# elfi-dev/elfi

Measured on NVIDIA H100. Metric: accepted particles/sec, higher is better.
Workload: dtype f64

## Files before the change

### elfi_b200/csrc/distance.cu

```cuda
#include <cstdlib>

#include "rowstream.cuh"

extern "C" int elfi_b200_colmoments_f64(elfi_b200_ctx* ctx, const double* S, int64_t ldS, int64_t B,
                                        int64_t D, double* out, void* stream);

namespace elfi {

struct DistParams {
    const double* obs;
    const double* W;
    double* d_out;
    uint32_t* mask;
    int K;
    int has_thr;
    const double* shift_src;
    double* mom_partial;
    const double* thr_dev;
    double thr[ELFI_B200_MAX_NESTED];
    __device__ __forceinline__ double threshold(int k) const {
        return thr_dev ? __ldg(thr_dev + k) : thr[k];
    }
};

__device__ __forceinline__ void dist_setup_shared(uint8_t* aux, const DistParams& p, int D,
                                                  bool weighted) {
    const int Dp = ((D + RS_BOX_COLS - 1) / RS_BOX_COLS) * RS_BOX_COLS;
    double* obs_s = reinterpret_cast<double*>(aux);
    for (int j = threadIdx.x; j < Dp; j += blockDim.x) obs_s[j] = j < D ? p.obs[j] : 0.0;
    if (weighted) {
        double* w_s = obs_s + Dp;
        for (int k = 0; k < p.K; ++k)
            for (int j = threadIdx.x; j < Dp; j += blockDim.x)
                w_s[size_t(k) * Dp + j] = j < D ? p.W[size_t(k) * D + j] : 0.0;
    }
}

template <int KMAX>
__device__ __forceinline__ void dist_finish(const DistParams& p, const double (&acc)[KMAX], int K,
                                            int64_t row, int64_t B, int lane) {
    bool ok = row < B;
    if (ok) {
#pragma unroll
        for (int k = 0; k < KMAX; ++k) {
            if (k < K) {
                const double d = sqrt(acc[k]);
                p.d_out[row * K + k] = d;
                if (p.has_thr) ok = ok && (d <= p.threshold(k));
            }
        }
    }
    if (p.mask != nullptr) {
        const uint32_t bits = __ballot_sync(0xffffffffu, ok && p.has_thr);
        if (lane == 0) p.mask[row >> 5] = bits;
    }
}

struct EuclidConsumer {
    typedef DistParams Params;
    static constexpr int PASSES = 1;
    const Params& p;
    const double* obs_s;
    double acc;

    static __device__ void setup_shared(uint8_t* aux, const Params& p, int D) {
        dist_setup_shared(aux, p, D, false);
    }
    __device__ EuclidConsumer(const Params& p_, const uint8_t* aux, int, int)
        : p(p_), obs_s(reinterpret_cast<const double*>(aux)), acc(0.0) {}
    __device__ __forceinline__ void begin_row() { acc = 0.0; }
    __device__ __forceinline__ void consume(int, int cg, const uint8_t* box_row, int sw) {
        const double2* o = reinterpret_cast<const double2*>(obs_s + cg * RS_BOX_COLS);
#pragma unroll
        for (int c = 0; c < 8; ++c) {
            const double2 v = *reinterpret_cast<const double2*>(box_row + ((c ^ sw) << 4));
            const double2 ob = o[c];
            const double d0 = __dsub_rn(v.x, ob.x);
            const double d1 = __dsub_rn(v.y, ob.y);
            acc = __dadd_rn(acc, __dmul_rn(d0, d0));
            acc = __dadd_rn(acc, __dmul_rn(d1, d1));
        }
    }
    __device__ __forceinline__ void end_row(int64_t row, int64_t B, int lane) {
        const double a1[1] = {acc};
        dist_finish<1>(p, a1, 1, row, B, lane);
    }
};

struct WeightedConsumer {
    typedef DistParams Params;
    static constexpr int PASSES = 1;
    const Params& p;
    const double* obs_s;
    const double* w_s;
    double acc;

    static __device__ void setup_shared(uint8_t* aux, const Params& p, int D) {
        dist_setup_shared(aux, p, D, true);
    }
    __device__ WeightedConsumer(const Params& p_, const uint8_t* aux, int D, int)
        : p(p_), obs_s(reinterpret_cast<const double*>(aux)), acc(0.0) {
        w_s = obs_s + ((D + RS_BOX_COLS - 1) / RS_BOX_COLS) * RS_BOX_COLS;
    }
    __device__ __forceinline__ void begin_row() { acc = 0.0; }
    __device__ __forceinline__ void consume(int, int cg, const uint8_t* box_row, int sw) {
        const double2* o = reinterpret_cast<const double2*>(obs_s + cg * RS_BOX_COLS);
        const double2* wv = reinterpret_cast<const double2*>(w_s + cg * RS_BOX_COLS);
#pragma unroll
        for (int c = 0; c < 8; ++c) {
            const double2 v = *reinterpret_cast<const double2*>(box_row + ((c ^ sw) << 4));
            const double2 ob = o[c];
            const double2 w = wv[c];
            const double d0 = __dsub_rn(v.x, ob.x);
            const double d1 = __dsub_rn(v.y, ob.y);
            acc = __dadd_rn(acc, __dmul_rn(w.x, __dmul_rn(d0, d0)));
            acc = __dadd_rn(acc, __dmul_rn(w.y, __dmul_rn(d1, d1)));
        }
    }
    __device__ __forceinline__ void end_row(int64_t row, int64_t B, int lane) {
        const double a1[1] = {acc};
        dist_finish<1>(p, a1, 1, row, B, lane);
    }
};

template <int KMAX>
struct NestedConsumer {
    typedef DistParams Params;
    static constexpr int PASSES = 1;
    const Params& p;
    const double* obs_s;
    const double* w_s;
    int Dp;
    double acc[KMAX];

    static __device__ void setup_shared(uint8_t* aux, const Params& p, int D) {
        dist_setup_shared(aux, p, D, true);
    }
    __device__ NestedConsumer(const Params& p_, const uint8_t* aux, int D, int)
        : p(p_), obs_s(reinterpret_cast<const double*>(aux)) {
        Dp = ((D + RS_BOX_COLS - 1) / RS_BOX_COLS) * RS_BOX_COLS;
        w_s = obs_s + Dp;
#pragma unroll
        for (int k = 0; k < KMAX; ++k) acc[k] = 0.0;
    }
    __device__ __forceinline__ void begin_row() {
#pragma unroll
        for (int k = 0; k < KMAX; ++k) acc[k] = 0.0;
    }
    __device__ __forceinline__ void consume(int, int cg, const uint8_t* box_row, int sw) {
        const double2* o = reinterpret_cast<const double2*>(obs_s + cg * RS_BOX_COLS);
        const int K = p.K;
#pragma unroll
        for (int c = 0; c < 8; ++c) {
            const double2 v = *reinterpret_cast<const double2*>(box_row + ((c ^ sw) << 4));
            const double2 ob = o[c];
            const double d0 = __dsub_rn(v.x, ob.x);
            const double d1 = __dsub_rn(v.y, ob.y);
            const double s0 = __dmul_rn(d0, d0);
            const double s1 = __dmul_rn(d1, d1);
#pragma unroll
            for (int k = 0; k < KMAX; ++k) {
                if (k < K) {
                    const double2 w = *reinterpret_cast<const double2*>(
                        w_s + size_t(k) * Dp + cg * RS_BOX_COLS + 2 * c);
                    acc[k] = __dadd_rn(acc[k], __dmul_rn(w.x, s0));
                    acc[k] = __dadd_rn(acc[k], __dmul_rn(w.y, s1));
                }
            }
        }
    }
    __device__ __forceinline__ void end_row(int64_t row, int64_t B, int lane) {
        dist_finish<KMAX>(p, acc, p.K, row, B, lane);
    }
};

template <int KMAX>
struct NestedMomentsConsumer : NestedConsumer<KMAX> {
    typedef NestedConsumer<KMAX> Base;
    typedef DistParams Params;
    static constexpr bool RS_TILE_INFO = true;
    static constexpr bool RS_FINISH = true;
    const double* shift_s;
    double* acc_s;
    int64_t row0, nrows;
    int D;

    static __host__ __device__ size_t aux_bytes(int64_t Dp, int64_t K, int warps = RS_WARPS) {
        return size_t(Dp) * 8 * (1 + K + 1 + 2 * warps);
    }
    static __device__ void setup_shared(uint8_t* aux, const Params& p, int D) {
        dist_setup_shared(aux, p, D, true);
        const int Dp = ((D + RS_BOX_COLS - 1) / RS_BOX_COLS) * RS_BOX_COLS;
        double* shift = reinterpret_cast<double*>(aux) + size_t(1 + p.K) * Dp;
        for (int j = threadIdx.x; j < Dp; j += blockDim.x) shift[j] = j < D ? p.shift_src[j] : 0.0;
        double* acc = shift + Dp;
        const int warps = blockDim.x >> 5;
        for (int j = threadIdx.x; j < 2 * warps * Dp; j += blockDim.x) acc[j] = 0.0;
    }
    __device__ NestedMomentsConsumer(const Params& p_, const uint8_t* aux, int D_, int lane)
        : Base(p_, aux, D_, lane), row0(0), nrows(0), D(D_) {
        shift_s = this->obs_s + size_t(1 + p_.K) * this->Dp;
        acc_s = const_cast<double*>(shift_s) + this->Dp + size_t(threadIdx.x >> 5) * 2 * this->Dp;
    }
    __device__ __forceinline__ void set_tile(int64_t r0, int64_t B) { row0 = r0; nrows = B; }
    __device__ __forceinline__ void consume(int pass, int cg, const uint8_t* box_row, int sw) {
        Base::consume(pass, cg, box_row, sw);
        const int lane = threadIdx.x & 31;
        const int c2 = lane & 7, h = lane >> 3;
        const uint8_t* box = box_row - lane * 128;
        const double2 sh = *reinterpret_cast<const double2*>(shift_s + cg * RS_BOX_COLS + 2 * c2);
        double s1x = 0.0, s1y = 0.0, s2x = 0.0, s2y = 0.0;
#pragma unroll
        for (int i = 0; i < 8; ++i) {
            const int r = h * 8 + i;
            const double2 v = *reinterpret_cast<const double2*>(box + r * 128 + ((c2 ^ i) << 4));
            if (row0 + r < nrows) {
                const double dx = v.x - sh.x, dy = v.y - sh.y;
                s1x += dx;
                s1y += dy;
                s2x = fma(dx, dx, s2x);
                s2y = fma(dy, dy, s2y);
            }
        }
#pragma unroll
        for (int o = 8; o <= 16; o <<= 1) {
            s1x += __shfl_xor_sync(0xffffffffu, s1x, o);
            s1y += __shfl_xor_sync(0xffffffffu, s1y, o);
            s2x += __shfl_xor_sync(0xffffffffu, s2x, o);
            s2y += __shfl_xor_sync(0xffffffffu, s2y, o);
        }
        if (lane < 8) {
            double2* a1 = reinterpret_cast<double2*>(acc_s + cg * RS_BOX_COLS + 2 * c2);
            double2* a2 = reinterpret_cast<double2*>(acc_s + this->Dp + cg * RS_BOX_COLS + 2 * c2);
            double2 t1 = *a1, t2 = *a2;
            t1.x += s1x; t1.y += s1y; t2.x += s2x; t2.y += s2y;
            *a1 = t1;
            *a2 = t2;
        }
    }
    __device__ __forceinline__ void finish(int64_t gw, int lane) {
        double* out = this->p.mom_partial + gw * 2 * int64_t(D);
        for (int j = lane; j < D; j += 32) {
            out[j] = acc_s[j];
            out[D + j] = acc_s[this->Dp + j];
        }
    }
};

__global__ void __launch_bounds__(1024)
colmoments_flush_kernel(const double* __restrict__ S, const double* __restrict__ partial,
                        int64_t nwarps, int64_t B, int64_t D, double* __restrict__ out) {
    __shared__ double r1[32][33], r2[32][33];
    const int tx = threadIdx.x, ty = threadIdx.y;
    const int64_t c = int64_t(blockIdx.x) * 32 + tx;
    double s1 = 0.0, s2 = 0.0;
    if (c < D)
        for (int64_t b = ty; b < nwarps; b += 32) {
            s1 += partial[(b * 2 + 0) * D + c];
            s2 += partial[(b * 2 + 1) * D + c];
        }
    r1[ty][tx] = s1;
    r2[ty][tx] = s2;
    __syncthreads();
    if (ty == 0 && c < D) {
        for (int k = 1; k < 32; ++k) { s1 += r1[k][tx]; s2 += r2[k][tx]; }
        const double n = double(B);
        out[c] = S[c] + s1 / n;
        out[D + c] = s2 - s1 * s1 / n;
    }
}

template <int KMAX>
static int fused_moments_warps(elfi_b200_ctx* ctx, int64_t Dp, int64_t K) {
    int warps = 12;
    if (const char* e = getenv("ELFI_B200_FUSED_WARPS")) warps = atoi(e);
    if (KMAX > 8 || warps != 12) return RS_WARPS;
    const size_t aux = NestedMomentsConsumer<KMAX>::aux_bytes(Dp, K, warps);
    return rs_pick_stages(ctx->smem_optin, aux, warps) >= 3 ? warps : RS_WARPS;
}

template <int KMAX>
static int launch_nested_moments(elfi_b200_ctx* ctx, const double* S, int64_t ldS, int64_t B,
                                 int64_t D, DistParams p, double* moments, cudaStream_t stream) {
    const int64_t Dp = ((D + RS_BOX_COLS - 1) / RS_BOX_COLS) * RS_BOX_COLS;
    const int warps = fused_moments_warps<KMAX>(ctx, Dp, p.K);
    const size_t aux = NestedMomentsConsumer<KMAX>::aux_bytes(Dp, p.K, warps);
    const int64_t ntiles = (B + RS_BOX_ROWS - 1) / RS_BOX_ROWS;
    int64_t ctas = (ntiles + warps - 1) / warps;
    if (ctas > ctx->sm_count) ctas = ctx->sm_count;
    const int64_t nwarps = ctas * warps;
    int rc;
    if constexpr (KMAX <= 8) {
        if (warps == 12)
            rc = rowstream_launch<NestedMomentsConsumer<KMAX>, 12>(ctx, S, ldS, B, D, aux, p, stream);
        else
            rc = rowstream_launch<NestedMomentsConsumer<KMAX>>(ctx, S, ldS, B, D, aux, p, stream);
    } else {
        rc = rowstream_launch<NestedMomentsConsumer<KMAX>>(ctx, S, ldS, B, D, aux, p, stream);
    }
    if (rc) return rc;
    colmoments_flush_kernel<<<unsigned((D + 31) / 32), dim3(32, 32), 0, stream>>>(
        S, p.mom_partial, nwarps, B, D, moments);
    ELFI_CUDA_OK(cudaGetLastError());
    return ELFI_B200_OK;
}

__global__ void __launch_bounds__(256)
dist_direct_kernel(const double* __restrict__ S, int64_t ld, int64_t B, int D, DistParams p) {
    const int64_t row = int64_t(blockIdx.x) * blockDim.x + threadIdx.x;
    const int lane = threadIdx.x & 31;
    const int K = p.K;
    bool ok = row < B;
    if (ok) {
        const double* r = S + row * ld;
        for (int k = 0; k < K; ++k) {
            double acc = 0.0;
            if (p.W != nullptr) {
                const double* w = p.W + size_t(k) * D;
                for (int j = 0; j < D; ++j) {
                    const double d = __dsub_rn(__ldg(r + j), __ldg(p.obs + j));
                    acc = __dadd_rn(acc, __dmul_rn(__ldg(w + j), __dmul_rn(d, d)));
                }
            } else {
                for (int j = 0; j < D; ++j) {
                    const double d = __dsub_rn(__ldg(r + j), __ldg(p.obs + j));
                    acc = __dadd_rn(acc, __dmul_rn(d, d));
                }
            }
            const double dist = sqrt(acc);
            p.d_out[row * K + k] = dist;
            if (p.has_thr) ok = ok && (dist <= p.threshold(k));
        }
    }
    if (p.mask != nullptr) {
        const uint32_t bits = __ballot_sync(0xffffffffu, ok && p.has_thr);
        if (lane == 0 && (row - lane) < B) p.mask[row >> 5] = bits;
    }
}

__global__ void __launch_bounds__(1024)
compact_mask_kernel(const uint32_t* __restrict__ mask, int64_t nwords, int64_t B,
                    int32_t* __restrict__ idx, int64_t* __restrict__ n_out) {
    __shared__ int64_t warp_sums[32];
    __shared__ int64_t base_s;
    const int tid = threadIdx.x;
    const int lane = tid & 31;
    const int wid = tid >> 5;
    const int64_t first = int64_t(blockIdx.x) * 1024;

    int64_t before = 0;
    for (int64_t w = tid; w < first; w += 1024) before += __popc(mask[w]);
    for (int o = 16; o > 0; o >>= 1) before += __shfl_xor_sync(0xffffffffu, before, o);
    if (lane == 0) warp_sums[wid] = before;
    __syncthreads();
    if (tid == 0) {
        int64_t t = 0;
        for (int i = 0; i < 32; ++i) t += warp_sums[i];
        base_s = t;
    }
    __syncthreads();
    const int64_t base = base_s;
    __syncthreads();

    const int64_t w = first + tid;
    const uint32_t bits = w < nwords ? mask[w] : 0u;
    const int cnt = __popc(bits);
    int incl = cnt;
    for (int o = 1; o < 32; o <<= 1) {
        const int t = __shfl_up_sync(0xffffffffu, incl, o);
        if (lane >= o) incl += t;
    }
    if (lane == 31) warp_sums[wid] = incl;
    __syncthreads();
    if (wid == 0) {
        int64_t v = warp_sums[lane];
        int64_t inc2 = v;
        for (int o = 1; o < 32; o <<= 1) {
            const int64_t t = __shfl_up_sync(0xffffffffu, inc2, o);
            if (lane >= o) inc2 += t;
        }
        warp_sums[lane] = inc2 - v;
        if (lane == 31 && blockIdx.x == gridDim.x - 1 && n_out != nullptr) *n_out = base + inc2;
    }
    __syncthreads();
    int64_t pos = base + warp_sums[wid] + (incl - cnt);
    if (idx != nullptr) {
        uint32_t b = bits;
        while (b) {
            const int bit = __ffs(b) - 1;
            b &= b - 1;
            idx[pos++] = int32_t(w * 32 + bit);
        }
    }
}

int launch_compact_mask(const uint32_t* mask, int64_t B, int32_t* idx, int64_t* n_out,
                        cudaStream_t stream) {
    const int64_t nwords = (B + 31) / 32;
    if (nwords == 0) {
        if (n_out) ELFI_CUDA_OK(cudaMemsetAsync(n_out, 0, sizeof(int64_t), stream));
        return ELFI_B200_OK;
    }
    const unsigned blocks = unsigned((nwords + 1023) / 1024);
    compact_mask_kernel<<<blocks, 1024, 0, stream>>>(mask, nwords, B, idx, n_out);
    ELFI_CUDA_OK(cudaGetLastError());
    return ELFI_B200_OK;
}

int launch_dist(elfi_b200_ctx* ctx, const double* S, int64_t ldS, int64_t B, int64_t D,
                const double* obs, const double* W, int64_t K, const double* thr_host,
                double* d_out, uint32_t* mask, cudaStream_t stream,
                const double* thr_dev = nullptr) {
    DistParams p;
    memset(&p, 0, sizeof(p));
    p.obs = obs;
    p.W = W;
    p.d_out = d_out;
    p.mask = mask;
    p.K = int(K);
    p.has_thr = thr_host != nullptr || thr_dev != nullptr;
    p.thr_dev = thr_dev;
    if (thr_host)
        for (int k = 0; k < K; ++k) p.thr[k] = thr_host[k];
    if (B == 0) return ELFI_B200_OK;

    const int64_t Dp = ((D + RS_BOX_COLS - 1) / RS_BOX_COLS) * RS_BOX_COLS;
    const bool use_tma = D >= RS_BOX_COLS && tma_compatible(S, ldS);
    if (use_tma) {
        const size_t aux = size_t(Dp) * 8 * (W ? (1 + K) : 1);
        if (rs_pick_stages(ctx->smem_optin, aux) >= 2) {
            if (W == nullptr) return rowstream_launch<EuclidConsumer>(ctx, S, ldS, B, D, aux, p, stream);
            if (K == 1) return rowstream_launch<WeightedConsumer>(ctx, S, ldS, B, D, aux, p, stream);
            if (K <= 2) return rowstream_launch<NestedConsumer<2>>(ctx, S, ldS, B, D, aux, p, stream);
            if (K <= 3) return rowstream_launch<NestedConsumer<3>>(ctx, S, ldS, B, D, aux, p, stream);
            if (K <= 4) return rowstream_launch<NestedConsumer<4>>(ctx, S, ldS, B, D, aux, p, stream);
            if (K <= 5) return rowstream_launch<NestedConsumer<5>>(ctx, S, ldS, B, D, aux, p, stream);
            if (K <= 6) return rowstream_launch<NestedConsumer<6>>(ctx, S, ldS, B, D, aux, p, stream);
            if (K <= 8) return rowstream_launch<NestedConsumer<8>>(ctx, S, ldS, B, D, aux, p, stream);
            if (K <= 16) return rowstream_launch<NestedConsumer<16>>(ctx, S, ldS, B, D, aux, p, stream);
            return rowstream_launch<NestedConsumer<32>>(ctx, S, ldS, B, D, aux, p, stream);
        }
    }
    const unsigned blocks = unsigned((B + 255) / 256);
    dist_direct_kernel<<<blocks, 256, 0, stream>>>(S, ldS, B, int(D), p);
    ELFI_CUDA_OK(cudaGetLastError());
    return ELFI_B200_OK;
}

struct MetricParams : DistParams {
    double pexp;
    const double* V;
};

template <int METRIC>
__device__ __forceinline__ double metric_term(double acc, double d, double pexp) {
    if (METRIC == ELFI_B200_METRIC_SQEUCLIDEAN) return __dadd_rn(acc, __dmul_rn(d, d));
    if (METRIC == ELFI_B200_METRIC_CITYBLOCK) return __dadd_rn(acc, fabs(d));
    if (METRIC == ELFI_B200_METRIC_CHEBYSHEV) return fabs(d) > acc ? fabs(d) : acc;
    return __dadd_rn(acc, pow(fabs(d), pexp));
}

template <int METRIC>
__device__ __forceinline__ double metric_value(double acc, double pexp) {
    return METRIC == ELFI_B200_METRIC_MINKOWSKI ? pow(acc, 1.0 / pexp) : acc;
}

template <int METRIC>
__device__ __forceinline__ void metric_finish(const MetricParams& p, double acc, int64_t row,
                                              int64_t B, int lane, bool whole_warp) {
    bool ok = row < B;
    if (ok) {
        const double d = metric_value<METRIC>(acc, p.pexp);
        p.d_out[row] = d;
        if (p.has_thr) ok = d <= p.threshold(0);
    }
    if (p.mask != nullptr) {
        const uint32_t bits = __ballot_sync(0xffffffffu, ok && p.has_thr);
        if (lane == 0 && (whole_warp || (row - lane) < B)) p.mask[row >> 5] = bits;
    }
}

template <int METRIC>
struct MetricConsumer {
    typedef MetricParams Params;
    static constexpr int PASSES = 1;
    const Params& p;
    const double* obs_s;
    double acc;

    static __device__ void setup_shared(uint8_t* aux, const Params& p, int D) {
        dist_setup_shared(aux, p, D, false);
    }
    __device__ MetricConsumer(const Params& p_, const uint8_t* aux, int, int)
        : p(p_), obs_s(reinterpret_cast<const double*>(aux)), acc(0.0) {}
    __device__ __forceinline__ void begin_row() { acc = 0.0; }
    __device__ __forceinline__ void consume(int, int cg, const uint8_t* box_row, int sw) {
        const double2* o = reinterpret_cast<const double2*>(obs_s + cg * RS_BOX_COLS);
#pragma unroll
        for (int c = 0; c < 8; ++c) {
            const double2 v = *reinterpret_cast<const double2*>(box_row + ((c ^ sw) << 4));
            const double2 ob = o[c];
            acc = metric_term<METRIC>(acc, __dsub_rn(v.x, ob.x), p.pexp);
            acc = metric_term<METRIC>(acc, __dsub_rn(v.y, ob.y), p.pexp);
        }
    }
    __device__ __forceinline__ void end_row(int64_t row, int64_t B, int lane) {
        metric_finish<METRIC>(p, acc, row, B, lane, true);
    }
};

template <int METRIC>
__global__ void __launch_bounds__(256)
metric_direct_kernel(const double* __restrict__ S, int64_t ld, int64_t B, int D, MetricParams p) {
    const int64_t row = int64_t(blockIdx.x) * blockDim.x + threadIdx.x;
    double acc = 0.0;
    if (row < B) {
        const double* r = S + row * ld;
        for (int j = 0; j < D; ++j)
            acc = metric_term<METRIC>(acc, __dsub_rn(__ldg(r + j), __ldg(p.obs + j)), p.pexp);
    }
    metric_finish<METRIC>(p, acc, row, B, threadIdx.x & 31, false);
}

template <int METRIC>
static int launch_metric_t(elfi_b200_ctx* ctx, const double* S, int64_t ldS, int64_t B, int64_t D,
                           const MetricParams& p, cudaStream_t stream) {
    const int64_t Dp = ((D + RS_BOX_COLS - 1) / RS_BOX_COLS) * RS_BOX_COLS;
    const size_t aux = size_t(Dp) * 8;
    if (D >= RS_BOX_COLS && tma_compatible(S, ldS) && rs_pick_stages(ctx->smem_optin, aux) >= 2)
        return rowstream_launch<MetricConsumer<METRIC>>(ctx, S, ldS, B, D, aux, p, stream);
    metric_direct_kernel<METRIC><<<unsigned((B + 255) / 256), 256, 0, stream>>>(S, ldS, B, int(D), p);
    ELFI_CUDA_OK(cudaGetLastError());
    return ELFI_B200_OK;
}

static int launch_metric(elfi_b200_ctx* ctx, int metric, double pexp, const double* S, int64_t ldS,
                         int64_t B, int64_t D, const double* obs, const double* thr_host,
                         double* d_out, uint32_t* mask, cudaStream_t stream) {
    MetricParams p;
    memset(&p, 0, sizeof(p));
    p.obs = obs;
    p.d_out = d_out;
    p.mask = mask;
    p.K = 1;
    p.has_thr = thr_host != nullptr;
    if (thr_host) p.thr[0] = thr_host[0];
    p.pexp = pexp;
    if (B == 0) return ELFI_B200_OK;
    switch (metric) {
        case ELFI_B200_METRIC_SQEUCLIDEAN:
            return launch_metric_t<ELFI_B200_METRIC_SQEUCLIDEAN>(ctx, S, ldS, B, D, p, stream);
        case ELFI_B200_METRIC_CITYBLOCK:
            return launch_metric_t<ELFI_B200_METRIC_CITYBLOCK>(ctx, S, ldS, B, D, p, stream);
        case ELFI_B200_METRIC_CHEBYSHEV:
            return launch_metric_t<ELFI_B200_METRIC_CHEBYSHEV>(ctx, S, ldS, B, D, p, stream);
        default:
            return launch_metric_t<ELFI_B200_METRIC_MINKOWSKI>(ctx, S, ldS, B, D, p, stream);
    }
}

struct SeuclidTerm {
    double even, odd, last;
    int j_last;
    __device__ __forceinline__ void begin(int D) {
        even = 0.0;
        odd = 0.0;
        last = 0.0;
        j_last = (D & 1) ? D - 1 : -1;
    }
    __device__ __forceinline__ void pair(int j0, double t0, double t1) {
        if (j0 == j_last) {
            last = t0;
        } else {
            even = __dadd_rn(even, t0);
            odd = __dadd_rn(odd, t1);
        }
    }
    __device__ __forceinline__ double value() const {
        const double s = __dadd_rn(even, odd);
        return sqrt(j_last >= 0 ? __dadd_rn(s, last) : s);
    }
};

__device__ __forceinline__ double seuclid_term(double x, double o, double v) {
    const double d = __dsub_rn(x, o);
    return __ddiv_rn(__dmul_rn(d, d), v);
}

__device__ __forceinline__ void seuclid_finish(const MetricParams& p, double dist, int64_t row,
                                               int64_t B, int lane, bool whole_warp) {
    bool ok = row < B;
    if (ok) {
        p.d_out[row] = dist;
        if (p.has_thr) ok = dist <= p.threshold(0);
    }
    if (p.mask != nullptr) {
        const uint32_t bits = __ballot_sync(0xffffffffu, ok && p.has_thr);
        if (lane == 0 && (whole_warp || (row - lane) < B)) p.mask[row >> 5] = bits;
    }
}

struct SeuclidConsumer {
    typedef MetricParams Params;
    static constexpr int PASSES = 1;
    const Params& p;
    const double* obs_s;
    const double* v_s;
    int D;
    SeuclidTerm acc;

    static __device__ void setup_shared(uint8_t* aux, const Params& p, int D) {
        const int Dp = ((D + RS_BOX_COLS - 1) / RS_BOX_COLS) * RS_BOX_COLS;
        double* obs_s = reinterpret_cast<double*>(aux);
        for (int j = threadIdx.x; j < Dp; j += blockDim.x) {
            obs_s[j] = j < D ? p.obs[j] : 0.0;
            obs_s[Dp + j] = j < D ? p.V[j] : 1.0;
        }
    }
    __device__ SeuclidConsumer(const Params& p_, const uint8_t* aux, int D_, int)
        : p(p_), obs_s(reinterpret_cast<const double*>(aux)), D(D_) {
        v_s = obs_s + ((D + RS_BOX_COLS - 1) / RS_BOX_COLS) * RS_BOX_COLS;
        acc.begin(D);
    }
    __device__ __forceinline__ void begin_row() { acc.begin(D); }
    __device__ __forceinline__ void consume(int, int cg, const uint8_t* box_row, int sw) {
        const double2* o = reinterpret_cast<const double2*>(obs_s + cg * RS_BOX_COLS);
        const double2* vv = reinterpret_cast<const double2*>(v_s + cg * RS_BOX_COLS);
#pragma unroll
        for (int c = 0; c < 8; ++c) {
            const double2 x = *reinterpret_cast<const double2*>(box_row + ((c ^ sw) << 4));
            const double2 ob = o[c];
            const double2 v = vv[c];
            acc.pair(cg * RS_BOX_COLS + 2 * c, seuclid_term(x.x, ob.x, v.x),
                     seuclid_term(x.y, ob.y, v.y));
        }
    }
    __device__ __forceinline__ void end_row(int64_t row, int64_t B, int lane) {
        seuclid_finish(p, acc.value(), row, B, lane, true);
    }
};

__global__ void __launch_bounds__(256)
seuclid_direct_kernel(const double* __restrict__ S, int64_t ld, int64_t B, int D, MetricParams p) {
    const int64_t row = int64_t(blockIdx.x) * blockDim.x + threadIdx.x;
    SeuclidTerm acc;
    acc.begin(D);
    if (row < B) {
        const double* r = S + row * ld;
        for (int j = 0; j < D; j += 2) {
            const double t0 = seuclid_term(__ldg(r + j), __ldg(p.obs + j), __ldg(p.V + j));
            const double t1 = j + 1 < D
                ? seuclid_term(__ldg(r + j + 1), __ldg(p.obs + j + 1), __ldg(p.V + j + 1)) : 0.0;
            acc.pair(j, t0, t1);
        }
    }
    seuclid_finish(p, acc.value(), row, B, threadIdx.x & 31, false);
}

static int launch_seuclid(elfi_b200_ctx* ctx, const double* S, int64_t ldS, int64_t B, int64_t D,
                          const double* obs, const double* V, const double* thr_host,
                          double* d_out, uint32_t* mask, cudaStream_t stream) {
    MetricParams p;
    memset(&p, 0, sizeof(p));
    p.obs = obs;
    p.V = V;
    p.d_out = d_out;
    p.mask = mask;
    p.K = 1;
    p.has_thr = thr_host != nullptr;
    if (thr_host) p.thr[0] = thr_host[0];
    if (B == 0) return ELFI_B200_OK;
    const int64_t Dp = ((D + RS_BOX_COLS - 1) / RS_BOX_COLS) * RS_BOX_COLS;
    const size_t aux = size_t(Dp) * 8 * 2;
    if (D >= RS_BOX_COLS && tma_compatible(S, ldS) && rs_pick_stages(ctx->smem_optin, aux) >= 2)
        return rowstream_launch<SeuclidConsumer>(ctx, S, ldS, B, D, aux, p, stream);
    seuclid_direct_kernel<<<unsigned((B + 255) / 256), 256, 0, stream>>>(S, ldS, B, int(D), p);
    ELFI_CUDA_OK(cudaGetLastError());
    return ELFI_B200_OK;
}

static int check_dist_args(const void* S, int64_t ldS, int64_t B, int64_t D, const void* obs,
                           const void* W, int64_t K, const void* thr, const void* acc_idx) {
    ELFI_REQUIRE(B >= 0 && D >= 1, "dist: bad shape B=%lld D=%lld", (long long)B, (long long)D);
    ELFI_REQUIRE(B == 0 || S != nullptr, "dist: S is NULL");
    ELFI_REQUIRE(obs != nullptr, "dist: obs is NULL");
    ELFI_REQUIRE(ldS >= D, "dist: ldS (%lld) < D (%lld)", (long long)ldS, (long long)D);
    ELFI_REQUIRE(K >= 1 && K <= ELFI_B200_MAX_NESTED, "dist: K=%lld outside [1, %d]",
                 (long long)K, ELFI_B200_MAX_NESTED);
    ELFI_REQUIRE(W != nullptr || K == 1, "dist: K=%lld needs a weight matrix", (long long)K);
    ELFI_REQUIRE(acc_idx == nullptr || thr != nullptr, "dist: acc_idx requires thresholds");
    ELFI_REQUIRE(B < (int64_t(1) << 31), "dist: B must fit int32 row indices");
    return ELFI_B200_OK;
}

}

extern "C" {

int elfi_b200_dist_euclid_thr_f64(elfi_b200_ctx* ctx, const double* S, int64_t ldS, int64_t B,
                                  int64_t D, const double* obs, const double* W, int64_t K,
                                  const double* thr_host, double* d_out, int32_t* acc_idx,
                                  int64_t* n_acc, void* stream_) {
    using namespace elfi;
    ELFI_REQUIRE(ctx != nullptr, "dist: ctx is NULL");
    int rc = check_dist_args(S, ldS, B, D, obs, W, K, thr_host, acc_idx);
    if (rc) return rc;
    ELFI_REQUIRE(B == 0 || d_out != nullptr, "dist: d_out is NULL");
    cudaStream_t stream = static_cast<cudaStream_t>(stream_);
    ELFI_CUDA_OK(cudaSetDevice(ctx->device));
    uint32_t* mask = nullptr;
    if (thr_host != nullptr) {
        const size_t nwords = size_t((B + 31) / 32);
        mask = static_cast<uint32_t*>(ctx_scratch(ctx, nwords * 4 + 256));
        if (!mask) return ELFI_B200_ERR_NOMEM;
    }
    rc = launch_dist(ctx, S, ldS, B, D, obs, W, K, thr_host, d_out, mask, stream);
    if (rc) return rc;
    if (thr_host != nullptr && (acc_idx != nullptr || n_acc != nullptr))
        return launch_compact_mask(mask, B, acc_idx, n_acc, stream);
    return ELFI_B200_OK;
}

int elfi_b200_dist_euclid_thr_dev_f64(elfi_b200_ctx* ctx, const double* S, int64_t ldS, int64_t B,
                                      int64_t D, const double* obs, const double* W, int64_t K,
                                      const double* thr_dev, double* d_out, int32_t* acc_idx,
                                      int64_t* n_acc, void* stream_) {
    using namespace elfi;
    ELFI_REQUIRE(ctx != nullptr && thr_dev != nullptr, "dist: ctx or thr_dev is NULL");
    int rc = check_dist_args(S, ldS, B, D, obs, W, K, thr_dev, acc_idx);
    if (rc) return rc;
    ELFI_REQUIRE(B == 0 || d_out != nullptr, "dist: d_out is NULL");
    cudaStream_t stream = static_cast<cudaStream_t>(stream_);
    ELFI_CUDA_OK(cudaSetDevice(ctx->device));
    const size_t nwords = size_t((B + 31) / 32);
    uint32_t* mask = static_cast<uint32_t*>(ctx_scratch(ctx, nwords * 4 + 256));
    if (!mask) return ELFI_B200_ERR_NOMEM;
    rc = launch_dist(ctx, S, ldS, B, D, obs, W, K, nullptr, d_out, mask, stream, thr_dev);
    if (rc) return rc;
    if (acc_idx != nullptr || n_acc != nullptr)
        return launch_compact_mask(mask, B, acc_idx, n_acc, stream);
    return ELFI_B200_OK;
}

int elfi_b200_dist_euclid_mom_f64(elfi_b200_ctx* ctx, const double* S, int64_t ldS, int64_t B,
                                  int64_t D, const double* obs, const double* W, int64_t K,
                                  const double* thr_host, const double* thr_dev, double* d_out,
                                  int32_t* acc_idx, int64_t* n_acc, double* moments,
                                  void* stream_) {
    using namespace elfi;
    ELFI_REQUIRE(ctx != nullptr && moments != nullptr, "dist_mom: ctx or moments is NULL");
    ELFI_REQUIRE(!(thr_host && thr_dev), "dist_mom: give thresholds on the host OR on the device");
    const void* thr = thr_host ? static_cast<const void*>(thr_host) : thr_dev;
    int rc = check_dist_args(S, ldS, B, D, obs, W, K, thr, acc_idx);
    if (rc) return rc;
    ELFI_REQUIRE(B >= 1 && d_out != nullptr, "dist_mom: needs at least one row and d_out");
    cudaStream_t stream = static_cast<cudaStream_t>(stream_);
    ELFI_CUDA_OK(cudaSetDevice(ctx->device));
    const int64_t Dp = ((D + RS_BOX_COLS - 1) / RS_BOX_COLS) * RS_BOX_COLS;
    const size_t aux = NestedMomentsConsumer<2>::aux_bytes(Dp, K);
    const bool fused = W != nullptr && D >= RS_BOX_COLS && tma_compatible(S, ldS) &&
                       rs_pick_stages(ctx->smem_optin, aux) >= 2;
    const size_t mask_bytes = (size_t((B + 31) / 32) * 4 + 255) & ~size_t(255);
    const size_t part_bytes = fused ? size_t(ctx->sm_count) * 16 * 2 * D * 8 : 0;
    uint8_t* base = static_cast<uint8_t*>(ctx_scratch(ctx, mask_bytes + part_bytes + 256));
    if (!base) return ELFI_B200_ERR_NOMEM;
    uint32_t* mask = thr ? reinterpret_cast<uint32_t*>(base) : nullptr;
    if (!fused) {
        rc = launch_dist(ctx, S, ldS, B, D, obs, W, K, thr_host, d_out, mask, stream, thr_dev);
        if (rc) return rc;
        if (thr && (acc_idx != nullptr || n_acc != nullptr)) {
            rc = launch_compact_mask(mask, B, acc_idx, n_acc, stream);
            if (rc) return rc;
        }
        return elfi_b200_colmoments_f64(ctx, S, ldS, B, D, moments, stream_);
    }
    DistParams p;
    memset(&p, 0, sizeof(p));
    p.obs = obs;
    p.W = W;
    p.d_out = d_out;
    p.mask = mask;
    p.K = int(K);
    p.has_thr = thr != nullptr;
    p.thr_dev = thr_dev;
    if (thr_host)
        for (int k = 0; k < K; ++k) p.thr[k] = thr_host[k];
    p.shift_src = S;
    p.mom_partial = reinterpret_cast<double*>(base + mask_bytes);
    if (K <= 2) rc = launch_nested_moments<2>(ctx, S, ldS, B, D, p, moments, stream);
    else if (K <= 4) rc = launch_nested_moments<4>(ctx, S, ldS, B, D, p, moments, stream);
    else if (K <= 6) rc = launch_nested_moments<6>(ctx, S, ldS, B, D, p, moments, stream);
    else if (K <= 8) rc = launch_nested_moments<8>(ctx, S, ldS, B, D, p, moments, stream);
    else if (K <= 16) rc = launch_nested_moments<16>(ctx, S, ldS, B, D, p, moments, stream);
    else rc = launch_nested_moments<32>(ctx, S, ldS, B, D, p, moments, stream);
    if (rc) return rc;
    if (thr && (acc_idx != nullptr || n_acc != nullptr))
        return launch_compact_mask(mask, B, acc_idx, n_acc, stream);
    return ELFI_B200_OK;
}

int elfi_b200_dist_euclid_thr_f64_host(elfi_b200_ctx* ctx, const double* S_host, int64_t ldS,
                                       int64_t B, int64_t D, const double* obs_host,
                                       const double* W_host, int64_t K, const double* thr_host,
                                       double* d_out_host, int32_t* acc_idx_host,
                                       int64_t* n_acc_host) {
    using namespace elfi;
    ELFI_REQUIRE(ctx != nullptr, "dist_host: ctx is NULL");
    int rc = check_dist_args(S_host, ldS, B, D, obs_host, W_host, K, thr_host, acc_idx_host);
    if (rc) return rc;
    ELFI_CUDA_OK(cudaSetDevice(ctx->device));

    const int64_t row_bytes = D * 8;
    int64_t chunk_rows = (int64_t(32) << 20) / row_bytes;
    chunk_rows = (chunk_rows / 32) * 32;
    if (chunk_rows < 32) chunk_rows = 32;
    if (chunk_rows > B) chunk_rows = ((B + 31) / 32) * 32;
    const size_t chunk_bytes = size_t(chunk_rows) * row_bytes;
    const size_t nwords = size_t((B + 31) / 32);
    auto align = [](size_t v) { return (v + 255) & ~size_t(255); };
    const size_t off_chunk1 = align(chunk_bytes);
    const size_t off_obs = off_chunk1 + align(chunk_bytes);
    const size_t off_w = off_obs + align(size_t(D) * 8);
    const size_t off_d = off_w + align(size_t(K) * D * 8);
    const size_t off_mask = off_d + align(size_t(B) * K * 8);
    const size_t off_idx = off_mask + align(nwords * 4 + 4);
    const size_t off_n = off_idx + align(size_t(B) * 4 + 4);
    const size_t total = off_n + 256;
    if (total > ctx->dev_stage_bytes) {
        ELFI_CUDA_OK(cudaDeviceSynchronize());
        if (ctx->dev_stage) ELFI_CUDA_OK(cudaFree(ctx->dev_stage));
        ctx->dev_stage = nullptr;
        ctx->dev_stage_bytes = 0;
        ELFI_CUDA_OK(cudaMalloc(&ctx->dev_stage, total));
        ctx->dev_stage_bytes = total;
    }
    uint8_t* base = static_cast<uint8_t*>(ctx->dev_stage);
    double* chunk[2] = {reinterpret_cast<double*>(base), reinterpret_cast<double*>(base + off_chunk1)};
    double* obs_d = reinterpret_cast<double*>(base + off_obs);
    double* w_d = W_host ? reinterpret_cast<double*>(base + off_w) : nullptr;
    double* d_d = reinterpret_cast<double*>(base + off_d);
    uint32_t* mask_d = thr_host ? reinterpret_cast<uint32_t*>(base + off_mask) : nullptr;
    int32_t* idx_d = reinterpret_cast<int32_t*>(base + off_idx);
    int64_t* n_d = reinterpret_cast<int64_t*>(base + off_n);

    cudaStream_t s0 = ctx->copy_stream[0], s1 = ctx->copy_stream[1];
    ELFI_CUDA_OK(cudaMemcpyAsync(obs_d, obs_host, size_t(D) * 8, cudaMemcpyHostToDevice, s0));
    if (W_host)
        ELFI_CUDA_OK(cudaMemcpyAsync(w_d, W_host, size_t(K) * D * 8, cudaMemcpyHostToDevice, s0));
    ELFI_CUDA_OK(cudaEventRecord(ctx->copy_event[0], s0));
    ELFI_CUDA_OK(cudaStreamWaitEvent(s1, ctx->copy_event[0], 0));

    int which = 0;
    for (int64_t r0 = 0; r0 < B; r0 += chunk_rows, which ^= 1) {
        const int64_t rows = (B - r0) < chunk_rows ? (B - r0) : chunk_rows;
        cudaStream_t st = which ? s1 : s0;
        if (ldS == D) {
            ELFI_CUDA_OK(cudaMemcpyAsync(chunk[which], S_host + r0 * ldS, size_t(rows) * row_bytes,
                                         cudaMemcpyHostToDevice, st));
        } else {
            ELFI_CUDA_OK(cudaMemcpy2DAsync(chunk[which], size_t(row_bytes), S_host + r0 * ldS,
                                           size_t(ldS) * 8, size_t(row_bytes), size_t(rows),
                                           cudaMemcpyHostToDevice, st));
        }
        rc = launch_dist(ctx, chunk[which], D, rows, D, obs_d, w_d, K, thr_host, d_d + r0 * K,
                         mask_d ? mask_d + r0 / 32 : nullptr, st);
        if (rc) return rc;
    }
    ELFI_CUDA_OK(cudaEventRecord(ctx->copy_event[1], s1));
    ELFI_CUDA_OK(cudaStreamWaitEvent(s0, ctx->copy_event[1], 0));
    ELFI_CUDA_OK(cudaEventRecord(ctx->copy_event[2], s0));
    ELFI_CUDA_OK(cudaStreamWaitEvent(s1, ctx->copy_event[2], 0));
    if (d_out_host && B > 0)
        ELFI_CUDA_OK(cudaMemcpyAsync(d_out_host, d_d, size_t(B) * K * 8, cudaMemcpyDeviceToHost, s1));
    int64_t n_acc = 0;
    if (thr_host != nullptr) {
        rc = launch_compact_mask(mask_d, B, acc_idx_host ? idx_d : nullptr, n_d, s0);
        if (rc) return rc;
        ELFI_CUDA_OK(cudaMemcpyAsync(&n_acc, n_d, 8, cudaMemcpyDeviceToHost, s0));
        ELFI_CUDA_OK(cudaStreamSynchronize(s0));
        if (acc_idx_host && n_acc > 0)
            ELFI_CUDA_OK(cudaMemcpyAsync(acc_idx_host, idx_d, size_t(n_acc) * 4,
                                         cudaMemcpyDeviceToHost, s0));
        if (n_acc_host) *n_acc_host = n_acc;
    }
    ELFI_CUDA_OK(cudaStreamSynchronize(s0));
    ELFI_CUDA_OK(cudaStreamSynchronize(s1));
    return ELFI_B200_OK;
}

int elfi_b200_dist_metric_thr_f64(elfi_b200_ctx* ctx, int32_t metric, double pexp, const double* S,
                                  int64_t ldS, int64_t B, int64_t D, const double* obs,
                                  const double* thr_host, double* d_out, int32_t* acc_idx,
                                  int64_t* n_acc, void* stream_) {
    using namespace elfi;
    ELFI_REQUIRE(ctx != nullptr, "dist_metric: ctx is NULL");
    ELFI_REQUIRE(metric >= ELFI_B200_METRIC_SQEUCLIDEAN && metric <= ELFI_B200_METRIC_MINKOWSKI,
                 "dist_metric: unknown metric code %d", int(metric));
    ELFI_REQUIRE(metric != ELFI_B200_METRIC_MINKOWSKI || (pexp > 0.0 && pexp < 1e308),
                 "dist_metric: Minkowski exponent must be positive and finite");
    int rc = check_dist_args(S, ldS, B, D, obs, nullptr, 1, thr_host, acc_idx);
    if (rc) return rc;
    ELFI_REQUIRE(B == 0 || d_out != nullptr, "dist_metric: d_out is NULL");
    cudaStream_t stream = static_cast<cudaStream_t>(stream_);
    ELFI_CUDA_OK(cudaSetDevice(ctx->device));
    uint32_t* mask = nullptr;
    if (thr_host != nullptr) {
        mask = static_cast<uint32_t*>(ctx_scratch(ctx, size_t((B + 31) / 32) * 4 + 256));
        if (!mask) return ELFI_B200_ERR_NOMEM;
    }
    rc = launch_metric(ctx, int(metric), pexp, S, ldS, B, D, obs, thr_host, d_out, mask, stream);
    if (rc) return rc;
    if (thr_host != nullptr && (acc_idx != nullptr || n_acc != nullptr))
        return launch_compact_mask(mask, B, acc_idx, n_acc, stream);
    return ELFI_B200_OK;
}

int elfi_b200_dist_seuclidean_thr_f64(elfi_b200_ctx* ctx, const double* S, int64_t ldS, int64_t B,
                                      int64_t D, const double* obs, const double* V,
                                      const double* thr_host, double* d_out, int32_t* acc_idx,
                                      int64_t* n_acc, void* stream_) {
    using namespace elfi;
    ELFI_REQUIRE(ctx != nullptr, "dist_seuclidean: ctx is NULL");
    ELFI_REQUIRE(V != nullptr, "dist_seuclidean: V is NULL");
    int rc = check_dist_args(S, ldS, B, D, obs, nullptr, 1, thr_host, acc_idx);
    if (rc) return rc;
    ELFI_REQUIRE(B == 0 || d_out != nullptr, "dist_seuclidean: d_out is NULL");
    cudaStream_t stream = static_cast<cudaStream_t>(stream_);
    ELFI_CUDA_OK(cudaSetDevice(ctx->device));
    uint32_t* mask = nullptr;
    if (thr_host != nullptr) {
        mask = static_cast<uint32_t*>(ctx_scratch(ctx, size_t((B + 31) / 32) * 4 + 256));
        if (!mask) return ELFI_B200_ERR_NOMEM;
    }
    rc = launch_seuclid(ctx, S, ldS, B, D, obs, V, thr_host, d_out, mask, stream);
    if (rc) return rc;
    if (thr_host != nullptr && (acc_idx != nullptr || n_acc != nullptr))
        return launch_compact_mask(mask, B, acc_idx, n_acc, stream);
    return ELFI_B200_OK;
}

}
```

### elfi_b200/csrc/rowstream.cuh

```cuda
#pragma once

#include <type_traits>

#include "common.cuh"

namespace elfi {

template <class C, class = void> struct rs_has_tile_info : std::false_type {};
template <class C> struct rs_has_tile_info<C, std::void_t<decltype(C::RS_TILE_INFO)>> : std::true_type {};
template <class C, class = void> struct rs_has_finish : std::false_type {};
template <class C> struct rs_has_finish<C, std::void_t<decltype(C::RS_FINISH)>> : std::true_type {};

constexpr int RS_WARPS = 8;
constexpr int RS_BOX_ROWS = 32;
constexpr int RS_BOX_COLS = 16;
constexpr int RS_BOX_BYTES = RS_BOX_ROWS * RS_BOX_COLS * 8;
constexpr int RS_MAX_STAGES = 6;

__host__ __device__ inline size_t rs_box_bytes(int ns, int warps = RS_WARPS) {
    return size_t(warps) * ns * RS_BOX_BYTES;
}
__host__ __device__ inline size_t rs_bar_bytes(int ns, int warps = RS_WARPS) {
    return size_t(warps) * ns * 8;
}
__host__ __device__ inline size_t rs_aux_offset(int ns, int warps = RS_WARPS) {
    return (rs_box_bytes(ns, warps) + rs_bar_bytes(ns, warps) + 15) & ~size_t(15);
}

inline int rs_pick_stages(size_t smem_optin, size_t aux_bytes, int warps = RS_WARPS) {
    for (int ns = RS_MAX_STAGES; ns >= 2; --ns)
        if (rs_aux_offset(ns, warps) + aux_bytes + 1024 <= smem_optin) return ns;
    return 0;
}

template <class Consumer, int WARPS = RS_WARPS>
__global__ void __launch_bounds__(WARPS * 32, 1)
rowstream_kernel(const __grid_constant__ CUtensorMap map, int64_t B, int D, int ns,
                 typename Consumer::Params params) {
    extern __shared__ __align__(1024) uint8_t smem[];
    const int warp = threadIdx.x >> 5;
    const int lane = threadIdx.x & 31;
    uint8_t* aux = smem + rs_aux_offset(ns, WARPS);

    Consumer::setup_shared(aux, params, D);

    const uint32_t box0 = smem_u32(smem) + uint32_t(warp) * ns * RS_BOX_BYTES;
    const uint32_t bar0 = smem_u32(smem + rs_box_bytes(ns, WARPS)) + uint32_t(warp) * ns * 8;
    const uint8_t* box0_generic = smem + size_t(warp) * ns * RS_BOX_BYTES;

    if (lane == 0) {
        if (warp == 0) tma_prefetch_desc(&map);
        for (int s = 0; s < ns; ++s) mbar_init(bar0 + s * 8, 1);
        mbar_fence_init();
    }
    __syncthreads();

    const int Gc = (D + RS_BOX_COLS - 1) / RS_BOX_COLS;
    const int G = Gc * Consumer::PASSES;
    const int64_t ntiles = (B + RS_BOX_ROWS - 1) / RS_BOX_ROWS;
    const int64_t gw = int64_t(blockIdx.x) * WARPS + warp;
    const int64_t GW = int64_t(gridDim.x) * WARPS;
    const int64_t my_tiles = gw < ntiles ? (ntiles - gw + GW - 1) / GW : 0;
    const int64_t nbox = my_tiles * G;

    int64_t p_tile = gw;
    int p_cg = 0;
    int p_col = 0;
    int64_t p_q = 0;
    int p_s = 0;
    auto issue = [&]() {
        mbar_arrive_expect_tx(bar0 + p_s * 8, RS_BOX_BYTES);
        tma_load_2d(box0 + p_s * RS_BOX_BYTES, &map, p_col * RS_BOX_COLS,
                    int32_t(p_tile * RS_BOX_ROWS), bar0 + p_s * 8);
        ++p_q;
        if (++p_s == ns) p_s = 0;
        if (++p_col == Gc) p_col = 0;
        if (++p_cg == G) { p_cg = 0; p_tile += GW; }
    };
    if (lane == 0) {
        const int64_t pre = nbox < ns ? nbox : ns;
        for (int64_t i = 0; i < pre; ++i) issue();
    }

    Consumer c(params, aux, D, lane);
    const int sw = lane & 7;
    const uint32_t row_off = uint32_t(lane) * 128;

    int s = 0;
    uint32_t parity = 0;
    int cg = 0;
    int col = 0;
    int pass = 0;
    int64_t tile = gw;
    for (int64_t q = 0; q < nbox; ++q) {
        mbar_wait(bar0 + s * 8, parity);
        if (cg == 0) {
            c.begin_row();
            if constexpr (rs_has_tile_info<Consumer>::value) c.set_tile(tile * RS_BOX_ROWS, B);
        }
        c.consume(pass, col, box0_generic + size_t(s) * RS_BOX_BYTES + row_off, sw);
        __syncwarp();
        if (lane == 0 && p_q < nbox) issue();
        if (cg == G - 1) c.end_row(tile * RS_BOX_ROWS + lane, B, lane);
        if (++col == Gc) { col = 0; ++pass; }
        if (++cg == G) { cg = 0; pass = 0; tile += GW; }
        if (++s == ns) { s = 0; parity ^= 1; }
    }
    if constexpr (rs_has_finish<Consumer>::value) {
        __syncwarp();
        c.finish(gw, lane);
    }
}

template <class Consumer, int WARPS = RS_WARPS>
int rowstream_launch(elfi_b200_ctx* ctx, const double* M, int64_t ld, int64_t B, int64_t D,
                     size_t aux_bytes, const typename Consumer::Params& params,
                     cudaStream_t stream) {
    ELFI_REQUIRE(D <= (int64_t(1) << 30) && B < (int64_t(1) << 31),
                 "matrix too large for int32 TMA coordinates (B=%lld, D=%lld)", (long long)B,
                 (long long)D);
    if (B == 0) return ELFI_B200_OK;
    const int ns = rs_pick_stages(ctx->smem_optin, aux_bytes, WARPS);
    ELFI_REQUIRE(ns >= 2, "row too wide for the shared-memory pipeline (D=%lld)", (long long)D);
    CUtensorMap map;
    int rc = make_rowmajor_f64_map(ctx, M, B, D, ld, RS_BOX_ROWS, &map);
    if (rc) return rc;
    const size_t smem_bytes = rs_aux_offset(ns, WARPS) + aux_bytes;
    auto kern = rowstream_kernel<Consumer, WARPS>;
    ELFI_CUDA_OK(cudaFuncSetAttribute(kern, cudaFuncAttributeMaxDynamicSharedMemorySize,
                                      int(smem_bytes)));
    const int64_t ntiles = (B + RS_BOX_ROWS - 1) / RS_BOX_ROWS;
    int64_t ctas = (ntiles + WARPS - 1) / WARPS;
    if (ctas > ctx->sm_count) ctas = ctx->sm_count;
    kern<<<dim3(unsigned(ctas)), dim3(WARPS * 32), smem_bytes, stream>>>(map, B, int(D), ns, params);
    ELFI_CUDA_OK(cudaGetLastError());
    return ELFI_B200_OK;
}

}
```

### elfi_b200/csrc/select.cu

```cuda
#include <cstdlib>

#include "eqweight.h"
#include "pairwise.cuh"

namespace elfi {

constexpr int SORT_CHUNK = 1024;
constexpr int SORT_WARPS = 8;

__device__ __forceinline__ uint64_t key_to_u64(double d) {
    if (d != d) return ~uint64_t(0);
    uint64_t u = static_cast<uint64_t>(__double_as_longlong(d));
    return (u >> 63) ? ~u : (u | (uint64_t(1) << 63));
}
__device__ __forceinline__ double u64_to_key(uint64_t u) {
    if (u == ~uint64_t(0)) return __longlong_as_double(0x7ff8000000000000LL);
    u = (u >> 63) ? (u & ~(uint64_t(1) << 63)) : ~u;
    return __longlong_as_double(static_cast<long long>(u));
}

__global__ void __launch_bounds__(256)
sort_prepare_kernel(const double* __restrict__ keys, int64_t n, uint64_t* __restrict__ ukeys,
                    int32_t* __restrict__ vals, uint32_t* __restrict__ ghist) {
    __shared__ uint32_t h[8 * 256];
    for (int i = threadIdx.x; i < 8 * 256; i += blockDim.x) h[i] = 0;
    __syncthreads();
    const int64_t stride = int64_t(gridDim.x) * blockDim.x;
    for (int64_t i = int64_t(blockIdx.x) * blockDim.x + threadIdx.x; i < n; i += stride) {
        const uint64_t u = key_to_u64(keys[i]);
        ukeys[i] = u;
        vals[i] = int32_t(i);
#pragma unroll
        for (int p = 0; p < 8; ++p) atomicAdd(&h[p * 256 + ((u >> (8 * p)) & 255)], 1u);
    }
    __syncthreads();
    for (int i = threadIdx.x; i < 8 * 256; i += blockDim.x)
        if (h[i]) atomicAdd(&ghist[i], h[i]);
}

__device__ __forceinline__ bool pass_trivial(const uint32_t* ghist, int pass, int64_t n,
                                             uint64_t first_key) {
    return ghist[pass * 256 + ((first_key >> (8 * pass)) & 255)] == uint32_t(n);
}

__global__ void __launch_bounds__(SORT_WARPS * 32)
sort_upsweep_kernel(const uint64_t* __restrict__ ukeys, int64_t n, int pass, int64_t nw,
                    const uint32_t* __restrict__ ghist, uint32_t* __restrict__ whist) {
    if (pass_trivial(ghist, pass, n, ukeys[0])) return;
    __shared__ uint32_t h[SORT_WARPS][256];
    const int warp = threadIdx.x >> 5, lane = threadIdx.x & 31;
    const int64_t gw = int64_t(blockIdx.x) * SORT_WARPS + warp;
    for (int i = lane; i < 256; i += 32) h[warp][i] = 0;
    __syncwarp();
    if (gw < nw) {
        const int64_t lo = gw * SORT_CHUNK;
        const int64_t hi = (lo + SORT_CHUNK < n) ? lo + SORT_CHUNK : n;
        for (int64_t i = lo + lane; i < hi; i += 32)
            atomicAdd(&h[warp][(ukeys[i] >> (8 * pass)) & 255], 1u);
        __syncwarp();
        for (int d = lane; d < 256; d += 32) whist[int64_t(d) * nw + gw] = h[warp][d];
    }
}

__global__ void __launch_bounds__(1024)
sort_scan_kernel(const uint64_t* __restrict__ ukeys, int64_t n, int pass, int64_t nw,
                 const uint32_t* __restrict__ ghist, uint32_t* __restrict__ whist) {
    if (pass_trivial(ghist, pass, n, ukeys[0])) return;
    __shared__ uint32_t warp_tot[32];
    __shared__ uint32_t carry_s;
    const int d = blockIdx.x;
    const int tid = threadIdx.x, lane = tid & 31, wid = tid >> 5;
    uint32_t part = 0;
    for (int i = tid; i < d; i += 1024) part += ghist[pass * 256 + i];
    for (int o = 16; o > 0; o >>= 1) part += __shfl_xor_sync(0xffffffffu, part, o);
    if (lane == 0) warp_tot[wid] = part;
    __syncthreads();
    if (tid == 0) {
        uint32_t t = 0;
        for (int i = 0; i < 32; ++i) t += warp_tot[i];
        carry_s = t;
    }
    __syncthreads();
    uint32_t* row = whist + int64_t(d) * nw;
    for (int64_t base = 0; base < nw; base += 1024) {
        const int64_t i = base + tid;
        const uint32_t v = i < nw ? row[i] : 0u;
        uint32_t incl = v;
        for (int o = 1; o < 32; o <<= 1) {
            const uint32_t t = __shfl_up_sync(0xffffffffu, incl, o);
            if (lane >= o) incl += t;
        }
        __syncthreads();
        if (lane == 31) warp_tot[wid] = incl;
        __syncthreads();
        uint32_t woff = 0;
        for (int k = 0; k < wid; ++k) woff += warp_tot[k];
        const uint32_t carry = carry_s;
        if (i < nw) row[i] = carry + woff + incl - v;
        __syncthreads();
        if (tid == 1023) carry_s = carry + woff + incl;
    }
}

__global__ void __launch_bounds__(SORT_WARPS * 32)
sort_scatter_kernel(const uint64_t* __restrict__ kin, const int32_t* __restrict__ vin, int64_t n,
                    int pass, int64_t nw, const uint32_t* __restrict__ ghist,
                    const uint32_t* __restrict__ whist, uint64_t* __restrict__ kout,
                    int32_t* __restrict__ vout) {
    const int warp = threadIdx.x >> 5, lane = threadIdx.x & 31;
    const int64_t gw = int64_t(blockIdx.x) * SORT_WARPS + warp;
    if (gw >= nw) return;
    const int64_t lo = gw * SORT_CHUNK;
    const int64_t hi = (lo + SORT_CHUNK < n) ? lo + SORT_CHUNK : n;
    if (pass_trivial(ghist, pass, n, kin[0])) {
        for (int64_t i = lo + lane; i < hi; i += 32) {
            kout[i] = kin[i];
            vout[i] = vin[i];
        }
        return;
    }
    __shared__ uint32_t off[SORT_WARPS][256];
    for (int d = lane; d < 256; d += 32) off[warp][d] = whist[int64_t(d) * nw + gw];
    __syncwarp();
    for (int64_t base = lo; base < hi; base += 32) {
        const int64_t i = base + lane;
        const bool valid = i < hi;
        const uint64_t k = valid ? kin[i] : 0;
        const int32_t v = valid ? vin[i] : 0;
        const uint32_t digit = valid ? uint32_t((k >> (8 * pass)) & 255) : 256u + lane;
        const uint32_t peers = __match_any_sync(0xffffffffu, digit);
        const uint32_t rank = __popc(peers & ((1u << lane) - 1));
        uint32_t pos = 0;
        if (valid) pos = off[warp][digit] + rank;
        __syncwarp();
        if (valid && rank == 0) off[warp][digit] += __popc(peers);
        __syncwarp();
        if (valid) {
            kout[pos] = k;
            vout[pos] = v;
        }
    }
}

__global__ void sort_finish_kernel(const uint64_t* __restrict__ ukeys, const int32_t* __restrict__ vals,
                                   int64_t n, double* __restrict__ keys_out,
                                   int32_t* __restrict__ perm_out) {
    const int64_t stride = int64_t(gridDim.x) * blockDim.x;
    for (int64_t i = int64_t(blockIdx.x) * blockDim.x + threadIdx.x; i < n; i += stride) {
        if (keys_out) keys_out[i] = u64_to_key(ukeys[i]);
        if (perm_out) perm_out[i] = vals[i];
    }
}

struct SortScratch {
    uint64_t* k[2];
    int32_t* v[2];
    uint32_t* ghist;
    uint32_t* whist;
    int64_t nw;
};

static size_t align256(size_t v) { return (v + 255) & ~size_t(255); }

static size_t sort_scratch_bytes(int64_t n) {
    const int64_t nw = (n + SORT_CHUNK - 1) / SORT_CHUNK;
    return 2 * align256(size_t(n) * 8) + 2 * align256(size_t(n) * 4) + align256(8 * 256 * 4) +
           align256(size_t(256) * nw * 4);
}

static SortScratch carve_sort(uint8_t* base, int64_t n) {
    SortScratch s;
    s.nw = (n + SORT_CHUNK - 1) / SORT_CHUNK;
    size_t o = 0;
    for (int i = 0; i < 2; ++i) { s.k[i] = reinterpret_cast<uint64_t*>(base + o); o += align256(size_t(n) * 8); }
    for (int i = 0; i < 2; ++i) { s.v[i] = reinterpret_cast<int32_t*>(base + o); o += align256(size_t(n) * 4); }
    s.ghist = reinterpret_cast<uint32_t*>(base + o); o += align256(8 * 256 * 4);
    s.whist = reinterpret_cast<uint32_t*>(base + o);
    return s;
}

int sort_pairs_device(const double* keys, int64_t n, const SortScratch& s, int sm_count,
                      cudaStream_t stream) {
    ELFI_CUDA_OK(cudaMemsetAsync(s.ghist, 0, 8 * 256 * 4, stream));
    int blocks = int((n + 256 * 8 - 1) / (256 * 8));
    if (blocks > sm_count * 4) blocks = sm_count * 4;
    if (blocks < 1) blocks = 1;
    sort_prepare_kernel<<<blocks, 256, 0, stream>>>(keys, n, s.k[0], s.v[0], s.ghist);
    const unsigned wblocks = unsigned((s.nw + SORT_WARPS - 1) / SORT_WARPS);
    int cur = 0;
    for (int pass = 0; pass < 8; ++pass) {
        sort_upsweep_kernel<<<wblocks, SORT_WARPS * 32, 0, stream>>>(s.k[cur], n, pass, s.nw, s.ghist, s.whist);
        sort_scan_kernel<<<256, 1024, 0, stream>>>(s.k[cur], n, pass, s.nw, s.ghist, s.whist);
        sort_scatter_kernel<<<wblocks, SORT_WARPS * 32, 0, stream>>>(
            s.k[cur], s.v[cur], n, pass, s.nw, s.ghist, s.whist, s.k[cur ^ 1], s.v[cur ^ 1]);
        cur ^= 1;
    }
    ELFI_CUDA_OK(cudaGetLastError());
    return ELFI_B200_OK;
}

__global__ void __launch_bounds__(256)
gather_rows_kernel(const double* __restrict__ src, int64_t ld_src, const int32_t* __restrict__ idx,
                   int64_t n, int64_t width, double* __restrict__ dst, int64_t ld_dst) {
    const int64_t total = n * width;
    const int64_t stride = int64_t(gridDim.x) * blockDim.x;
    for (int64_t t = int64_t(blockIdx.x) * blockDim.x + threadIdx.x; t < total; t += stride) {
        const int64_t i = t / width, j = t - i * width;
        dst[i * ld_dst + j] = src[int64_t(idx[i]) * ld_src + j];
    }
}

constexpr int APPEND_MAX_SRC = 8;
struct AppendSources {
    const double* ptr[APPEND_MAX_SRC];
    int64_t ld[APPEND_MAX_SRC];
    int32_t width[APPEND_MAX_SRC];
    int32_t col0[APPEND_MAX_SRC];
    int32_t n_src, total_width;
};

__global__ void __launch_bounds__(256)
accept_append_kernel(const int32_t* __restrict__ acc_idx, const int64_t* __restrict__ n_acc,
                     AppendSources src, double* __restrict__ dst, int64_t ld_dst, int64_t capacity,
                     const int64_t* __restrict__ count) {
    const int64_t base = *count;
    int64_t room = capacity - base;
    if (room < 0) room = 0;
    const int64_t rows = *n_acc < room ? *n_acc : room;
    const int64_t total = rows * src.total_width;
    const int64_t stride = int64_t(gridDim.x) * blockDim.x;
    for (int64_t t = int64_t(blockIdx.x) * blockDim.x + threadIdx.x; t < total; t += stride) {
        const int64_t j = t / src.total_width;
        const int c = int(t - j * src.total_width);
        const int64_t row = acc_idx ? int64_t(acc_idx[j]) : j;
        int k = 0;
#pragma unroll
        for (int q = 1; q < APPEND_MAX_SRC; ++q)
            if (q < src.n_src && c >= src.col0[q]) k = q;
        dst[(base + j) * ld_dst + c] = src.ptr[k][row * src.ld[k] + (c - src.col0[k])];
    }
}

__global__ void accept_count_kernel(const int64_t* __restrict__ n_acc, int64_t capacity,
                                    int64_t* __restrict__ count, int64_t* __restrict__ dropped) {
    int64_t room = capacity - *count;
    if (room < 0) room = 0;
    const int64_t rows = *n_acc < room ? *n_acc : room;
    if (dropped) *dropped += *n_acc - rows;
    *count += rows;
}

__global__ void __launch_bounds__(256)
gather2_rows_kernel(const double* __restrict__ A, int64_t ldA, int64_t nA,
                    const double* __restrict__ Bm, int64_t ldB, const int32_t* __restrict__ mapB,
                    const int32_t* __restrict__ perm, int64_t n, int64_t width,
                    double* __restrict__ dst, int64_t ld_dst) {
    const int64_t total = n * width;
    const int64_t stride = int64_t(gridDim.x) * blockDim.x;
    for (int64_t t = int64_t(blockIdx.x) * blockDim.x + threadIdx.x; t < total; t += stride) {
        const int64_t i = t / width, j = t - i * width;
        const int64_t r = perm ? perm[i] : i;
        double v;
        if (r < nA) {
            v = A[r * ldA + j];
        } else {
            const int64_t rb = mapB ? int64_t(mapB[r - nA]) : (r - nA);
            v = Bm[rb * ldB + j];
        }
        dst[i * ld_dst + j] = v;
    }
}

__global__ void __launch_bounds__(256)
merge_keys_kernel(const double* __restrict__ keysA, int64_t ldA, int64_t nA,
                  const double* __restrict__ keysB, int64_t ldB, const int32_t* __restrict__ mapB,
                  int64_t nB, double* __restrict__ out) {
    const int64_t stride = int64_t(gridDim.x) * blockDim.x;
    for (int64_t i = int64_t(blockIdx.x) * blockDim.x + threadIdx.x; i < nA + nB; i += stride) {
        if (i < nA) {
            out[i] = keysA[i * ldA];
        } else {
            const int64_t rb = mapB ? int64_t(mapB[i - nA]) : (i - nA);
            out[i] = keysB[rb * ldB];
        }
    }
}

constexpr int WQ_CHUNK = 1024;

__device__ __forceinline__ void wq_stage(const double* __restrict__ src, int64_t n, int64_t base,
                                         double* buf, int lane) {
    for (int t = lane; t < WQ_CHUNK; t += 32) {
        const int64_t i = base + t;
        buf[t] = i < n ? src[i] : 0.0;
    }
}

__global__ void __launch_bounds__(32)
wq_total_kernel(const double* __restrict__ w, int64_t n64, double* __restrict__ out) {
    __shared__ double buf[2][WQ_CHUNK];
    __shared__ double left_val[32];
    __shared__ int pending_right[32];
    const int lane = threadIdx.x;
    const int n = int(n64);
    if (w == nullptr) {
        if (lane == 0) out[0] = double(n);
        return;
    }
    uint32_t has_left = 0;
    int depth = 0, leaf_start = 0, leaf_end = 0, tail_start = 0;
    bool in_tail = false;
    double r = 0.0, res = 0.0;
    auto descend = [&](int start, int len) {
        while (len > 128) {
            int n2 = len / 2;
            n2 -= n2 % 8;
            if (lane == 0) pending_right[depth] = len - n2;
            has_left &= ~(1u << depth);
            ++depth;
            len = n2;
        }
        __syncwarp();
        leaf_start = start;
        leaf_end = start + len;
        tail_start = len < 8 ? start : start + (len - len % 8);
        in_tail = len < 8;
        res = 0.0;
    };
    auto fold = [&]() -> double {
        double t = r + __shfl_down_sync(0xffffffffu, r, 1);
        t = t + __shfl_down_sync(0xffffffffu, t, 2);
        t = t + __shfl_down_sync(0xffffffffu, t, 4);
        return __shfl_sync(0xffffffffu, t, 0);
    };
    auto leaf_value = [&]() -> double { return in_tail ? res : fold(); };
    descend(0, n);
    wq_stage(w, n64, 0, buf[0], lane);
    __syncwarp();
    int cur = 0;
    for (int base = 0; base < n; base += WQ_CHUNK, cur ^= 1) {
        if (int64_t(base) + WQ_CHUNK < n64) wq_stage(w, n64, int64_t(base) + WQ_CHUNK, buf[cur ^ 1], lane);
        const int lim = (n - base) < WQ_CHUNK ? (n - base) : WQ_CHUNK;
        for (int j = 0; j < lim; j += 8) {
            const int j0 = base + j;
            const int cnt = (lim - j) < 8 ? (lim - j) : 8;
            if (j0 == leaf_end) {
                double v = leaf_value();
                bool opened = false;
                while (depth > 0 && !opened) {
                    if (!((has_left >> (depth - 1)) & 1u)) {
                        if (lane == 0) left_val[depth - 1] = v;
                        has_left |= 1u << (depth - 1);
                        __syncwarp();
                        descend(j0, pending_right[depth - 1]);
                        opened = true;
                    } else {
                        v = left_val[depth - 1] + v;
                        --depth;
                    }
                }
            }
            if (!in_tail && j0 == tail_start && tail_start != leaf_start) {
                res = fold();
                in_tail = true;
            }
            if (in_tail) {
                for (int k = 0; k < cnt; ++k) res = res + buf[cur][j + k];
            } else if (lane < 8) {
                const double t = buf[cur][j + lane];
                r = (j0 == leaf_start) ? t : r + t;
            }
        }
        __syncwarp();
    }
    double v = leaf_value();
    while (depth > 0) {
        v = left_val[depth - 1] + v;
        --depth;
    }
    if (lane == 0) out[0] = v;
}

__global__ void wq_normalise_kernel(const double* __restrict__ w, const int32_t* __restrict__ perm,
                                    int64_t n, const double* __restrict__ total,
                                    double* __restrict__ ws) {
    const double t = total[0];
    const int64_t stride = int64_t(gridDim.x) * blockDim.x;
    for (int64_t i = int64_t(blockIdx.x) * blockDim.x + threadIdx.x; i < n; i += stride)
        ws[i] = (w ? w[perm[i]] : 1.0) / t;
}

__global__ void __launch_bounds__(32)
wq_seqscan_kernel(const double* __restrict__ ws, int64_t n, double alpha,
                  const uint64_t* __restrict__ ukeys, double* __restrict__ out) {
    __shared__ double buf[2][WQ_CHUNK];
    __shared__ int done_s;
    const int lane = threadIdx.x;
    int64_t count = 0;
    double c = 0.0;
    if (lane == 0) done_s = (alpha == 0.0) ? 1 : 0;
    wq_stage(ws, n, 0, buf[0], lane);
    __syncwarp();
    int cur = 0;
    for (int64_t base = 0; base < n - 1; base += WQ_CHUNK, cur ^= 1) {
        if (done_s) break;
        if (base + WQ_CHUNK < n - 1) wq_stage(ws, n, base + WQ_CHUNK, buf[cur ^ 1], lane);
        if (lane == 0) {
            const int lim = int((n - 1 - base) < WQ_CHUNK ? (n - 1 - base) : WQ_CHUNK);
            int j = 0;
            for (; j + 8 <= lim; j += 8) {
                double t[8];
#pragma unroll
                for (int k = 0; k < 8; ++k) t[k] = buf[cur][j + k];
                int below = 0;
#pragma unroll
                for (int k = 0; k < 8; ++k) {
                    c = __dadd_rn(c, t[k]);
                    below += (c < alpha) ? 1 : 0;
                }
                count += below;
                if (below < 8) { done_s = 1; break; }
            }
            if (!done_s) {
                for (; j < lim; ++j) {
                    c = __dadd_rn(c, buf[cur][j]);
                    if (c < alpha) ++count; else { done_s = 1; break; }
                }
            }
        }
        __syncwarp();
    }
    if (lane == 0) {
        out[0] = u64_to_key(ukeys[count]);
        out[1] = double(count);
    }
}

__global__ void __launch_bounds__(256)
rowsort_kernel(const double* __restrict__ X, int64_t ldX, int64_t B, int n, int npow2,
               double* __restrict__ out, int64_t ld_out) {
    extern __shared__ uint64_t sk_all[];
    const int warp = threadIdx.x >> 5, lane = threadIdx.x & 31;
    uint64_t* sk = sk_all + size_t(warp) * npow2;
    for (int64_t row = int64_t(blockIdx.x) * 8 + warp; row < B; row += int64_t(gridDim.x) * 8) {
        for (int i = lane; i < npow2; i += 32) sk[i] = i < n ? key_to_u64(X[row * ldX + i]) : ~uint64_t(0);
        __syncwarp();
        for (int k = 2; k <= npow2; k <<= 1) {
            for (int j = k >> 1; j > 0; j >>= 1) {
                for (int t = lane; t < (npow2 >> 1); t += 32) {
                    const int i = ((t & ~(j - 1)) << 1) | (t & (j - 1));
                    const int l = i | j;
                    const bool up = (i & k) == 0;
                    const uint64_t a = sk[i], b = sk[l];
                    if ((a > b) == up) { sk[i] = b; sk[l] = a; }
                }
                __syncwarp();
            }
        }
        for (int i = lane; i < n; i += 32) out[row * ld_out + i] = u64_to_key(sk[i]);
        __syncwarp();
    }
}

__device__ __forceinline__ uint64_t shfl_xor_u64(uint64_t v, int m) {
    uint32_t lo = uint32_t(v), hi = uint32_t(v >> 32);
    asm volatile("shfl.sync.bfly.b32 %0, %0, %2, 0x1f, 0xffffffff;\n\t"
                 "shfl.sync.bfly.b32 %1, %1, %2, 0x1f, 0xffffffff;"
                 : "+r"(lo), "+r"(hi) : "r"(m));
    return (uint64_t(hi) << 32) | lo;
}

template <int KPL>
__device__ __forceinline__ void bitonic_in_registers(uint64_t (&key)[KPL], int lane) {
    constexpr int N = KPL * 32;
#pragma unroll
    for (int k = 2; k <= N; k <<= 1) {
        const bool lane_up = (k >= N) ? true : ((lane & (k >= KPL ? k / KPL : 1)) == 0);
#pragma unroll
        for (int j = k >> 1; j > 0; j >>= 1) {
            if (j >= KPL) {
                const int m = j / KPL;
                const bool keep_min = ((lane & m) == 0) == lane_up;
#pragma unroll
                for (int r = 0; r < KPL; ++r) {
                    const uint64_t o = shfl_xor_u64(key[r], m);
                    key[r] = ((o < key[r]) == keep_min) ? o : key[r];
                }
            } else {
#pragma unroll
                for (int r = 0; r < KPL; ++r) {
                    if ((r & j) == 0) {
                        const bool up = (k < KPL) ? ((r & k) == 0) : lane_up;
                        const uint64_t a = key[r], b = key[r | j];
                        const bool sw = (a > b) == up;
                        key[r] = sw ? b : a;
                        key[r | j] = sw ? a : b;
                    }
                }
            }
        }
    }
}

template <int KPL>
__global__ void __launch_bounds__(256)
rowsort_regs_kernel(const double* __restrict__ X, int64_t ldX, int64_t B, int n_,
                    double* __restrict__ out, int64_t ld_out, int vec_in, int vec_out) {
    const int lane = threadIdx.x & 31;
    const int64_t nwarps = int64_t(gridDim.x) * 8;
    const int first = lane * KPL;
    for (int64_t base = int64_t(blockIdx.x) * 8; base < B; base += nwarps) {
        const int64_t row = base + (threadIdx.x >> 5);
        const bool live = row < B;
        const int n = live ? n_ : 0;
        const bool whole = first + KPL <= n;
        uint64_t key[KPL];
        const double* x = X + row * ldX + first;
        bool loaded = false;
        if constexpr (KPL >= 2) {
            if (vec_in && whole) {
#pragma unroll
                for (int r = 0; r < KPL; r += 2) {
                    const double2 v = __ldg(reinterpret_cast<const double2*>(x + r));
                    key[r] = key_to_u64(v.x);
                    key[r + 1] = key_to_u64(v.y);
                }
                loaded = true;
            }
        }
        if (!loaded) {
#pragma unroll
            for (int r = 0; r < KPL; ++r)
                key[r] = first + r < n ? key_to_u64(__ldg(x + r)) : ~uint64_t(0);
        }
        bitonic_in_registers<KPL>(key, lane);
        double* y = out + row * ld_out + first;
        bool stored = false;
        if constexpr (KPL >= 2) {
            if (vec_out && whole) {
#pragma unroll
                for (int r = 0; r < KPL; r += 2)
                    *reinterpret_cast<double2*>(y + r) =
                        make_double2(u64_to_key(key[r]), u64_to_key(key[r + 1]));
                stored = true;
            }
        }
        if (!stored) {
#pragma unroll
            for (int r = 0; r < KPL; ++r)
                if (first + r < n) y[r] = u64_to_key(key[r]);
        }
    }
}

template <int KPL>
static void launch_rowsort_regs(const double* X, int64_t ldX, int64_t B, int n, double* out,
                                int64_t ld_out, int sm_count, cudaStream_t stream) {
    int64_t blocks = (B + 7) / 8;
    if (blocks > int64_t(sm_count) * 8) blocks = int64_t(sm_count) * 8;
    const int vec_in = (reinterpret_cast<uintptr_t>(X) % 16 == 0) && (ldX % 2 == 0);
    const int vec_out = (reinterpret_cast<uintptr_t>(out) % 16 == 0) && (ld_out % 2 == 0);
    rowsort_regs_kernel<KPL><<<unsigned(blocks), 256, 0, stream>>>(X, ldX, B, n, out, ld_out,
                                                                   vec_in, vec_out);
}

__global__ void __launch_bounds__(1024)
wq_par_block_sums_kernel(const double* __restrict__ w, const int32_t* __restrict__ perm, int64_t n,
                         double* __restrict__ partial) {
    __shared__ double ws[32];
    const int64_t lo = int64_t(blockIdx.x) * 4096;
    double acc = 0.0;
    for (int k = 0; k < 4; ++k) {
        const int64_t i = lo + k * 1024 + threadIdx.x;
        if (i < n) acc += w ? w[perm[i]] : 1.0;
    }
    for (int o = 16; o > 0; o >>= 1) acc += __shfl_xor_sync(0xffffffffu, acc, o);
    if ((threadIdx.x & 31) == 0) ws[threadIdx.x >> 5] = acc;
    __syncthreads();
    if (threadIdx.x < 32) {
        double v = ws[threadIdx.x];
        for (int o = 16; o > 0; o >>= 1) v += __shfl_xor_sync(0xffffffffu, v, o);
        if (threadIdx.x == 0) partial[blockIdx.x] = v;
    }
}

__global__ void __launch_bounds__(1024)
wq_par_scan_kernel(double* __restrict__ partial, int64_t nb, int32_t* __restrict__ counts) {
    __shared__ double ws[32];
    __shared__ double carry_s;
    const int tid = threadIdx.x, lane = tid & 31, wid = tid >> 5;
    if (tid == 0) { carry_s = 0.0; counts[0] = 0; counts[1] = 0; }
    __syncthreads();
    for (int64_t base = 0; base < nb; base += 1024) {
        const int64_t i = base + tid;
        const double v = i < nb ? partial[i] : 0.0;
        double incl = v;
        for (int o = 1; o < 32; o <<= 1) {
            const double t = __shfl_up_sync(0xffffffffu, incl, o);
            if (lane >= o) incl += t;
        }
        if (lane == 31) ws[wid] = incl;
        __syncthreads();
        double woff = 0.0;
        for (int k = 0; k < wid; ++k) woff += ws[k];
        const double carry = carry_s;
        if (i < nb) partial[i] = carry + woff + incl - v;
        __syncthreads();
        if (tid == 1023) carry_s = carry + woff + incl;
        __syncthreads();
    }
    if (tid == 0) partial[nb] = carry_s;
}

__global__ void __launch_bounds__(1024)
wq_par_count_kernel(const double* __restrict__ w, const int32_t* __restrict__ perm, int64_t n,
                    const double* __restrict__ partial, int64_t nb, double alpha, double eps,
                    int32_t* __restrict__ counts) {
    __shared__ double ws[32];
    __shared__ double carry_s;
    __shared__ int c0_s, c1_s;
    const int tid = threadIdx.x, lane = tid & 31, wid = tid >> 5;
    const double total = partial[nb];
    if (tid == 0) { carry_s = partial[blockIdx.x]; c0_s = 0; c1_s = 0; }
    __syncthreads();
    int l0 = 0, l1 = 0;
    const int64_t lo = int64_t(blockIdx.x) * 4096;
    for (int k = 0; k < 4; ++k) {
        const int64_t i = lo + k * 1024 + tid;
        const double v = i < n ? (w ? w[perm[i]] : 1.0) : 0.0;
        double incl = v;
        for (int o = 1; o < 32; o <<= 1) {
            const double t = __shfl_up_sync(0xffffffffu, incl, o);
            if (lane >= o) incl += t;
        }
        if (lane == 31) ws[wid] = incl;
        __syncthreads();
        double woff = 0.0;
        for (int q = 0; q < wid; ++q) woff += ws[q];
        const double carry = carry_s;
        const double c = (carry + woff + incl) / total;
        if (i < n - 1) {
            l0 += (c < alpha - eps) ? 1 : 0;
            l1 += (c < alpha + eps) ? 1 : 0;
        }
        __syncthreads();
        if (tid == 1023) carry_s = carry + woff + incl;
        __syncthreads();
    }
    for (int o = 16; o > 0; o >>= 1) {
        l0 += __shfl_xor_sync(0xffffffffu, l0, o);
        l1 += __shfl_xor_sync(0xffffffffu, l1, o);
    }
    if (lane == 0) { atomicAdd(&c0_s, l0); atomicAdd(&c1_s, l1); }
    __syncthreads();
    if (tid == 0) { atomicAdd(&counts[0], c0_s); atomicAdd(&counts[1], c1_s); }
}

__global__ void wq_pick_kernel(const uint64_t* __restrict__ ukeys, int64_t idx, double* __restrict__ out) {
    out[0] = u64_to_key(ukeys[idx]);
    out[1] = double(idx);
}

}

extern "C" {

int elfi_b200_sort_pairs_f64(elfi_b200_ctx* ctx, const double* keys, int64_t n,
                             double* keys_sorted, int32_t* perm, void* stream_) {
    using namespace elfi;
    ELFI_REQUIRE(ctx != nullptr, "sort: ctx is NULL");
    ELFI_REQUIRE(n >= 0 && n < (int64_t(1) << 31), "sort: n=%lld out of range", (long long)n);
    if (n == 0) return ELFI_B200_OK;
    ELFI_REQUIRE(keys != nullptr, "sort: keys is NULL");
    cudaStream_t stream = static_cast<cudaStream_t>(stream_);
    ELFI_CUDA_OK(cudaSetDevice(ctx->device));
    uint8_t* base = static_cast<uint8_t*>(ctx_scratch(ctx, sort_scratch_bytes(n)));
    if (!base) return ELFI_B200_ERR_NOMEM;
    SortScratch s = carve_sort(base, n);
    int rc = sort_pairs_device(keys, n, s, ctx->sm_count, stream);
    if (rc) return rc;
    int blocks = int((n + 255) / 256);
    if (blocks > ctx->sm_count * 8) blocks = ctx->sm_count * 8;
    sort_finish_kernel<<<blocks, 256, 0, stream>>>(s.k[0], s.v[0], n, keys_sorted, perm);
    ELFI_CUDA_OK(cudaGetLastError());
    return ELFI_B200_OK;
}

int elfi_b200_gather_rows_f64(elfi_b200_ctx* ctx, const double* src, int64_t ld_src,
                              const int32_t* idx, int64_t n, int64_t width, double* dst,
                              int64_t ld_dst, void* stream_) {
    using namespace elfi;
    ELFI_REQUIRE(ctx != nullptr, "gather: ctx is NULL");
    ELFI_REQUIRE(n >= 0 && width >= 1 && ld_src >= width && ld_dst >= width, "gather: bad shape");
    if (n == 0) return ELFI_B200_OK;
    ELFI_REQUIRE(src && idx && dst, "gather: NULL argument");
    cudaStream_t stream = static_cast<cudaStream_t>(stream_);
    ELFI_CUDA_OK(cudaSetDevice(ctx->device));
    int64_t blocks = (n * width + 255) / 256;
    if (blocks > int64_t(ctx->sm_count) * 16) blocks = int64_t(ctx->sm_count) * 16;
    gather_rows_kernel<<<unsigned(blocks), 256, 0, stream>>>(src, ld_src, idx, n, width, dst, ld_dst);
    ELFI_CUDA_OK(cudaGetLastError());
    return ELFI_B200_OK;
}

int elfi_b200_gather2_rows_f64(elfi_b200_ctx* ctx, const double* A, int64_t ldA, int64_t nA,
                               const double* Bm, int64_t ldB, const int32_t* mapB,
                               const int32_t* perm, int64_t n, int64_t width, double* dst,
                               int64_t ld_dst, void* stream_) {
    using namespace elfi;
    ELFI_REQUIRE(ctx != nullptr, "gather2: ctx is NULL");
    ELFI_REQUIRE(n >= 0 && nA >= 0 && width >= 1 && ld_dst >= width, "gather2: bad shape");
    if (n == 0) return ELFI_B200_OK;
    ELFI_REQUIRE(dst != nullptr && (nA == 0 || A != nullptr), "gather2: NULL argument");
    cudaStream_t stream = static_cast<cudaStream_t>(stream_);
    ELFI_CUDA_OK(cudaSetDevice(ctx->device));
    int64_t blocks = (n * width + 255) / 256;
    if (blocks > int64_t(ctx->sm_count) * 16) blocks = int64_t(ctx->sm_count) * 16;
    gather2_rows_kernel<<<unsigned(blocks), 256, 0, stream>>>(A, ldA, nA, Bm, ldB, mapB, perm, n,
                                                             width, dst, ld_dst);
    ELFI_CUDA_OK(cudaGetLastError());
    return ELFI_B200_OK;
}

int elfi_b200_topn_merge_f64(elfi_b200_ctx* ctx, const double* keysA, int64_t ld_keysA, int64_t nA,
                             const double* keysB, int64_t ld_keysB, const int32_t* mapB, int64_t nB,
                             int64_t n_keep, int64_t n_out, const double* const* A_host,
                             const int64_t* ldA_host, const double* const* B_host,
                             const int64_t* ldB_host, const int64_t* width_host,
                             double* const* dst_host, const int64_t* ld_dst_host, void* stream_) {
    using namespace elfi;
    ELFI_REQUIRE(ctx != nullptr, "topn_merge: ctx is NULL");
    ELFI_REQUIRE(nA >= 0 && nB >= 0 && n_keep >= 0 && n_keep <= nA + nB && n_out >= 0,
                 "topn_merge: bad sizes (nA=%lld nB=%lld n_keep=%lld)", (long long)nA, (long long)nB,
                 (long long)n_keep);
    const int64_t n = nA + nB;
    ELFI_REQUIRE(n < (int64_t(1) << 31), "topn_merge: too many rows");
    if (n == 0 || n_keep == 0) return ELFI_B200_OK;
    ELFI_REQUIRE((nA == 0 || keysA) && (nB == 0 || keysB), "topn_merge: keys are NULL");
    ELFI_REQUIRE(n_out == 0 || (A_host && ldA_host && B_host && ldB_host && width_host && dst_host &&
                                ld_dst_host), "topn_merge: output descriptors are NULL");
    cudaStream_t stream = static_cast<cudaStream_t>(stream_);
    ELFI_CUDA_OK(cudaSetDevice(ctx->device));
    const size_t sort_bytes = sort_scratch_bytes(n);
    uint8_t* base = static_cast<uint8_t*>(ctx_scratch(ctx, sort_bytes + align256(size_t(n) * 8) + 256));
    if (!base) return ELFI_B200_ERR_NOMEM;
    SortScratch s = carve_sort(base, n);
    double* keys = reinterpret_cast<double*>(base + sort_bytes);
    int blocks = int((n + 255) / 256);
    if (blocks > ctx->sm_count * 8) blocks = ctx->sm_count * 8;
    merge_keys_kernel<<<blocks, 256, 0, stream>>>(keysA, ld_keysA, nA, keysB, ld_keysB, mapB, nB, keys);
    int rc = sort_pairs_device(keys, n, s, ctx->sm_count, stream);
    if (rc) return rc;
    const int32_t* perm = s.v[0];
    for (int64_t k = 0; k < n_out; ++k) {
        const int64_t width = width_host[k];
        ELFI_REQUIRE(width >= 1 && dst_host[k] && ld_dst_host[k] >= width &&
                     (nA == 0 || (A_host[k] && ldA_host[k] >= width)) &&
                     (nB == 0 || (B_host[k] && ldB_host[k] >= width)),
                     "topn_merge: bad descriptor of output %lld", (long long)k);
        int64_t gb = (n_keep * width + 255) / 256;
        if (gb > int64_t(ctx->sm_count) * 16) gb = int64_t(ctx->sm_count) * 16;
        gather2_rows_kernel<<<unsigned(gb), 256, 0, stream>>>(A_host[k], ldA_host[k], nA, B_host[k],
                                                              ldB_host[k], mapB, perm, n_keep, width,
                                                              dst_host[k], ld_dst_host[k]);
    }
    ELFI_CUDA_OK(cudaGetLastError());
    return ELFI_B200_OK;
}

int elfi_b200_accept_append_f64(elfi_b200_ctx* ctx, const int32_t* acc_idx, const int64_t* n_acc,
                                int64_t max_rows, int64_t n_src, const double* const* src_host,
                                const int64_t* ld_src_host, const int64_t* width_host, double* dst,
                                int64_t ld_dst, int64_t capacity, int64_t* count, int64_t* dropped,
                                void* stream_) {
    using namespace elfi;
    ELFI_REQUIRE(ctx && n_acc && src_host && ld_src_host && width_host && dst && count,
                 "accept_append: NULL argument");
    ELFI_REQUIRE(n_src >= 1 && n_src <= APPEND_MAX_SRC, "accept_append: 1..%d sources", APPEND_MAX_SRC);
    ELFI_REQUIRE(max_rows >= 0 && capacity >= 0, "accept_append: bad shape");
    AppendSources src;
    memset(&src, 0, sizeof(src));
    src.n_src = int32_t(n_src);
    int64_t col = 0;
    for (int k = 0; k < n_src; ++k) {
        ELFI_REQUIRE(src_host[k] && width_host[k] >= 1 && ld_src_host[k] >= width_host[k],
                     "accept_append: bad source %d", k);
        src.ptr[k] = src_host[k];
        src.ld[k] = ld_src_host[k];
        src.width[k] = int32_t(width_host[k]);
        src.col0[k] = int32_t(col);
        col += width_host[k];
    }
    ELFI_REQUIRE(col <= ld_dst && col < (int64_t(1) << 30), "accept_append: ld_dst < total width");
    src.total_width = int32_t(col);
    if (max_rows == 0) return ELFI_B200_OK;
    cudaStream_t stream = static_cast<cudaStream_t>(stream_);
    ELFI_CUDA_OK(cudaSetDevice(ctx->device));
    int64_t blocks = (max_rows * col + 255) / 256;
    if (blocks > int64_t(ctx->sm_count) * 8) blocks = int64_t(ctx->sm_count) * 8;
    accept_append_kernel<<<unsigned(blocks), 256, 0, stream>>>(acc_idx, n_acc, src, dst, ld_dst,
                                                              capacity, count);
    accept_count_kernel<<<1, 1, 0, stream>>>(n_acc, capacity, count, dropped);
    ELFI_CUDA_OK(cudaGetLastError());
    return ELFI_B200_OK;
}

extern "C" int elfi_b200_dist_euclid_thr_f64(elfi_b200_ctx*, const double*, int64_t, int64_t, int64_t,
                                             const double*, const double*, int64_t, const double*,
                                             double*, int32_t*, int64_t*, void*);
extern "C" int elfi_b200_dist_euclid_thr_dev_f64(elfi_b200_ctx*, const double*, int64_t, int64_t,
                                                 int64_t, const double*, const double*, int64_t,
                                                 const double*, double*, int32_t*, int64_t*, void*);

int elfi_b200_rejection_batch_f64(elfi_b200_ctx* ctx, const double* S, int64_t ldS, int64_t B,
                                  int64_t D, const double* obs, const double* W, int64_t K,
                                  const double* thr_host, const double* thr_dev, double* d_out,
                                  int32_t* acc_idx, int64_t* n_acc, int64_t n_extra,
                                  const double* const* extra_host, const int64_t* ld_extra_host,
                                  const int64_t* width_extra_host, double* dst, int64_t ld_dst,
                                  int64_t capacity, int64_t* count, int64_t* dropped,
                                  void* stream_) {
    using namespace elfi;
    ELFI_REQUIRE(ctx && acc_idx && n_acc && d_out, "rejection_batch: NULL argument");
    ELFI_REQUIRE((thr_host != nullptr) != (thr_dev != nullptr),
                 "rejection_batch: thresholds on the host OR on the device");
    ELFI_REQUIRE(n_extra >= 0 && n_extra < APPEND_MAX_SRC, "rejection_batch: 0..%d extra sources",
                 APPEND_MAX_SRC - 1);
    int rc = thr_host
        ? elfi_b200_dist_euclid_thr_f64(ctx, S, ldS, B, D, obs, W, K, thr_host, d_out, acc_idx, n_acc,
                                        stream_)
        : elfi_b200_dist_euclid_thr_dev_f64(ctx, S, ldS, B, D, obs, W, K, thr_dev, d_out, acc_idx,
                                            n_acc, stream_);
    if (rc) return rc;
    const double* src[APPEND_MAX_SRC];
    int64_t ld[APPEND_MAX_SRC], width[APPEND_MAX_SRC];
    src[0] = d_out; ld[0] = K; width[0] = K;
    for (int64_t k = 0; k < n_extra; ++k) {
        src[k + 1] = extra_host[k];
        ld[k + 1] = ld_extra_host[k];
        width[k + 1] = width_extra_host[k];
    }
    return elfi_b200_accept_append_f64(ctx, acc_idx, n_acc, B, n_extra + 1, src, ld, width, dst,
                                       ld_dst, capacity, count, dropped, stream_);
}

int elfi_b200_wquantile_f64(elfi_b200_ctx* ctx, const double* x, const double* w, int64_t n,
                            double alpha, double* out, void* stream_) {
    using namespace elfi;
    ELFI_REQUIRE(ctx != nullptr && x != nullptr && out != nullptr, "wquantile: NULL argument");
    ELFI_REQUIRE(n >= 1 && n < (int64_t(1) << 31), "wquantile: n=%lld out of range", (long long)n);
    ELFI_REQUIRE(alpha >= 0.0 && alpha <= 1.0, "wquantile: alpha=%g outside [0, 1]", alpha);
    cudaStream_t stream = static_cast<cudaStream_t>(stream_);
    ELFI_CUDA_OK(cudaSetDevice(ctx->device));
    const size_t sort_bytes = sort_scratch_bytes(n);
    const size_t extra = align256(size_t(n + 2) * 8) + 256;
    uint8_t* base = static_cast<uint8_t*>(ctx_scratch(ctx, sort_bytes + extra));
    if (!base) return ELFI_B200_ERR_NOMEM;
    SortScratch s = carve_sort(base, n);
    double* ws = reinterpret_cast<double*>(base + sort_bytes);
    double* total = reinterpret_cast<double*>(base + sort_bytes + align256(size_t(n) * 8));
    int rc = sort_pairs_device(x, n, s, ctx->sm_count, stream);
    if (rc) return rc;
    if (w == nullptr && alpha > 0.0) {
        wq_pick_kernel<<<1, 1, 0, stream>>>(s.k[0], equal_weight_cum_index(n, alpha) - 1, out);
        ELFI_CUDA_OK(cudaGetLastError());
        return ELFI_B200_OK;
    }
    if (alpha > 0.0 && n > 1) {
        const int64_t nb = (n + 4095) / 4096;
        double* partial = ws;
        int32_t* counts = reinterpret_cast<int32_t*>(total) + 4;
        const double eps = (4.0 * double(n) + 64.0) * 1.1102230246251565e-16;
        wq_par_block_sums_kernel<<<unsigned(nb), 1024, 0, stream>>>(w, s.v[0], n, partial);
        wq_par_scan_kernel<<<1, 1024, 0, stream>>>(partial, nb, counts);
        wq_par_count_kernel<<<unsigned(nb), 1024, 0, stream>>>(w, s.v[0], n, partial, nb, alpha, eps, counts);
        int32_t hc[2] = {0, -1};
        ELFI_CUDA_OK(cudaMemcpyAsync(hc, counts, 8, cudaMemcpyDeviceToHost, stream));
        ELFI_CUDA_OK(cudaStreamSynchronize(stream));
        if (hc[0] == hc[1]) {
            wq_pick_kernel<<<1, 1, 0, stream>>>(s.k[0], int64_t(hc[0]), out);
            ELFI_CUDA_OK(cudaGetLastError());
            return ELFI_B200_OK;
        }
    }
    wq_total_kernel<<<1, 32, 0, stream>>>(w, n, total);
    int blocks = int((n + 255) / 256);
    if (blocks > ctx->sm_count * 8) blocks = ctx->sm_count * 8;
    wq_normalise_kernel<<<blocks, 256, 0, stream>>>(w, s.v[0], n, total, ws);
    wq_seqscan_kernel<<<1, 32, 0, stream>>>(ws, n, alpha, s.k[0], out);
    ELFI_CUDA_OK(cudaGetLastError());
    return ELFI_B200_OK;
}

int elfi_b200_rowsort_f64(elfi_b200_ctx* ctx, const double* X, int64_t ldX, int64_t B, int64_t n,
                          double* out, int64_t ld_out, void* stream_) {
    using namespace elfi;
    ELFI_REQUIRE(ctx && (B == 0 || (X && out)), "rowsort: NULL argument");
    ELFI_REQUIRE(B >= 0 && n >= 1 && n <= 2048 && ldX >= n && ld_out >= n,
                 "rowsort: bad shape (1 <= n <= 2048)");
    if (B == 0) return ELFI_B200_OK;
    cudaStream_t stream = static_cast<cudaStream_t>(stream_);
    ELFI_CUDA_OK(cudaSetDevice(ctx->device));
    int npow2 = 2;
    while (npow2 < n) npow2 <<= 1;
    if (npow2 <= 512 && getenv("ELFI_B200_ROWSORT_SMEM") == nullptr) {
        const int kpl = npow2 <= 32 ? 1 : npow2 / 32;
        switch (kpl) {
            case 1: launch_rowsort_regs<1>(X, ldX, B, int(n), out, ld_out, ctx->sm_count, stream); break;
            case 2: launch_rowsort_regs<2>(X, ldX, B, int(n), out, ld_out, ctx->sm_count, stream); break;
            case 4: launch_rowsort_regs<4>(X, ldX, B, int(n), out, ld_out, ctx->sm_count, stream); break;
            case 8: launch_rowsort_regs<8>(X, ldX, B, int(n), out, ld_out, ctx->sm_count, stream); break;
            default: launch_rowsort_regs<16>(X, ldX, B, int(n), out, ld_out, ctx->sm_count, stream); break;
        }
        ELFI_CUDA_OK(cudaGetLastError());
        return ELFI_B200_OK;
    }
    const size_t smem = size_t(8) * npow2 * 8;
    ELFI_CUDA_OK(cudaFuncSetAttribute(rowsort_kernel, cudaFuncAttributeMaxDynamicSharedMemorySize,
                                      int(smem)));
    int64_t blocks = (B + 7) / 8;
    if (blocks > int64_t(ctx->sm_count) * 8) blocks = int64_t(ctx->sm_count) * 8;
    rowsort_kernel<<<unsigned(blocks), 256, smem, stream>>>(X, ldX, B, int(n), npow2, out, ld_out);
    ELFI_CUDA_OK(cudaGetLastError());
    return ELFI_B200_OK;
}

}
```

### elfi_b200/ops.py

```python
import ctypes

import numpy as np
import torch

from . import _lib
from . import device as dev

MAX_NESTED = 32


def _matrix(S):
    if dev.is_device_array(S) and S.dtype == torch.float64 and S.dim() == 2 \
            and S.stride(1) == 1 and S.stride(0) >= S.shape[1]:
        return S
    S = dev.to_device(S)
    if S.dim() == 1:
        S = S[:, None]
    if S.dim() != 2:
        raise ValueError('expected a 2-d (batch, dim) array, got shape {}'.format(tuple(S.shape)))
    if S.stride(1) != 1:
        S = S.contiguous()
    return S


def dist_euclid(S, obs, w=None, thresholds=None, want_indices=True, sync=True, moments=False):
    S = _matrix(S)
    B, D = S.shape
    obs_t = dev.to_device(obs).reshape(-1)
    if obs_t.numel() != D:
        raise ValueError('XA and XB must have the same number of columns '
                         '(i.e. feature dimension.)')
    squeeze = True
    W = None
    K = 1
    if w is not None:
        W = dev.to_device(w)
        if W.dim() == 1:
            W = W[None, :]
        else:
            squeeze = False
        K = W.shape[0]
        if W.shape[1] != D:
            raise ValueError('weights must have {} columns'.format(D))
        if K > MAX_NESTED:
            raise ValueError('at most {} nested distances are supported'.format(MAX_NESTED))
    thr = None
    thr_on_device = dev.is_device_array(thresholds)
    if thr_on_device:
        thr = thresholds.reshape(-1)
        if thr.dtype != torch.float64 or not thr.is_contiguous():
            thr = thr.to(torch.float64).contiguous()
    elif thresholds is not None:
        thr = np.ascontiguousarray(np.atleast_1d(thresholds), dtype=np.float64)
    if thr is not None and thr.shape[0] != K:
        raise ValueError('need one threshold per distance column ({} != {})'.format(
            thr.shape[0], K))
    d = dev.empty((B, K))
    acc_idx = n_acc = None
    if thr is not None:
        n_acc = dev.zeros((1,), dtype=torch.int64)
        if want_indices:
            acc_idx = dev.empty((max(B, 1),), dtype=torch.int32)
    mom = None
    if moments:
        mom = dev.empty((2, D))
        _lib.call('elfi_b200_dist_euclid_mom_f64', dev.context(), dev.ptr(S),
                  S.stride(0) if B > 1 else D, B, D, dev.ptr(obs_t), dev.ptr(W), K,
                  None if thr_on_device else dev.ptr(thr), dev.ptr(thr) if thr_on_device else None,
                  dev.ptr(d), dev.ptr(acc_idx), dev.ptr(n_acc), dev.ptr(mom), dev.stream_ptr())
    else:
        _lib.call('elfi_b200_dist_euclid_thr_dev_f64' if thr_on_device else
                  'elfi_b200_dist_euclid_thr_f64', dev.context(), dev.ptr(S),
                  S.stride(0) if B > 1 else D, B, D, dev.ptr(obs_t), dev.ptr(W), K, dev.ptr(thr),
                  dev.ptr(d), dev.ptr(acc_idx), dev.ptr(n_acc), dev.stream_ptr())
    if thr is not None:
        if not sync:
            acc_idx = (acc_idx, n_acc)
        else:
            n = int(n_acc.item())
            acc_idx = acc_idx[:n] if want_indices else n
    if squeeze:
        d = d.reshape(B)
    return (d, acc_idx, mom) if moments else (d, acc_idx)


METRIC_CODES = {'sqeuclidean': 1, 'cityblock': 2, 'chebyshev': 3, 'minkowski': 4}


def dist_metric(S, obs, metric, p=2.0, threshold=None, want_indices=True):
    if metric == 'minkowski':
        if p == 1:
            metric = 'cityblock'
        elif p == 2:
            return dist_euclid(S, obs, thresholds=threshold, want_indices=want_indices)
        elif np.isinf(p):
            metric = 'chebyshev'
        elif not p > 0:
            raise ValueError('p must be greater than 0')
    if metric not in METRIC_CODES:
        raise ValueError('Unknown Distance Metric: {}'.format(metric))
    S = _matrix(S)
    B, D = S.shape
    obs_t = dev.to_device(obs).reshape(-1)
    if obs_t.numel() != D:
        raise ValueError('XA and XB must have the same number of columns '
                         '(i.e. feature dimension.)')
    thr = None
    if threshold is not None:
        thr = np.ascontiguousarray(np.atleast_1d(threshold), dtype=np.float64)
        if thr.shape[0] != 1:
            raise ValueError('need one threshold per distance column ({} != 1)'.format(thr.shape[0]))
    d = dev.empty((B,))
    acc_idx = n_acc = None
    if thr is not None:
        n_acc = dev.zeros((1,), dtype=torch.int64)
        if want_indices:
            acc_idx = dev.empty((max(B, 1),), dtype=torch.int32)
    _lib.call('elfi_b200_dist_metric_thr_f64', dev.context(), METRIC_CODES[metric], float(p),
              dev.ptr(S), S.stride(0) if B > 1 else D, B, D, dev.ptr(obs_t), dev.ptr(thr),
              dev.ptr(d), dev.ptr(acc_idx), dev.ptr(n_acc), dev.stream_ptr())
    if thr is not None:
        n = int(n_acc.item())
        acc_idx = acc_idx[:n] if want_indices else n
    return d, acc_idx


def dist_seuclidean(S, obs, V, threshold=None, want_indices=True):
    S = _matrix(S)
    B, D = S.shape
    obs_t = dev.to_device(obs).reshape(-1)
    if obs_t.numel() != D:
        raise ValueError('XA and XB must have the same number of columns '
                         '(i.e. feature dimension.)')
    V_t = dev.to_device(V)
    if V_t.dim() != 1 or V_t.shape[0] != D:
        raise ValueError('Variance vector V must be of the same dimension as the vectors on '
                         'which the distances are computed.')
    thr = None
    if threshold is not None:
        thr = np.ascontiguousarray(np.atleast_1d(threshold), dtype=np.float64)
        if thr.shape[0] != 1:
            raise ValueError('need one threshold per distance column ({} != 1)'.format(thr.shape[0]))
    d = dev.empty((B,))
    acc_idx = n_acc = None
    if thr is not None:
        n_acc = dev.zeros((1,), dtype=torch.int64)
        if want_indices:
            acc_idx = dev.empty((max(B, 1),), dtype=torch.int32)
    _lib.call('elfi_b200_dist_seuclidean_thr_f64', dev.context(), dev.ptr(S),
              S.stride(0) if B > 1 else D, B, D, dev.ptr(obs_t), dev.ptr(V_t), dev.ptr(thr),
              dev.ptr(d), dev.ptr(acc_idx), dev.ptr(n_acc), dev.stream_ptr())
    if thr is not None:
        n = int(n_acc.item())
        acc_idx = acc_idx[:n] if want_indices else n
    return d, acc_idx


def dist_euclid_host(S, obs, w=None, thresholds=None, return_distances=True):
    S = np.asarray(S, dtype=np.float64)
    if S.ndim == 1:
        S = S[:, None]
    if S.strides[1] != 8:
        S = np.ascontiguousarray(S)
    B, D = S.shape
    ld = S.strides[0] // 8 if B > 1 else D
    obs = np.ascontiguousarray(obs, dtype=np.float64).reshape(-1)
    K = 1
    W = None
    if w is not None:
        W = np.ascontiguousarray(np.atleast_2d(w), dtype=np.float64)
        K = W.shape[0]
    thr = None if thresholds is None else np.ascontiguousarray(np.atleast_1d(thresholds),
                                                               dtype=np.float64)
    d = np.empty((B, K)) if return_distances else None
    idx = np.empty(max(B, 1), dtype=np.int32) if thr is not None else None
    n = ctypes.c_int64(0)
    _lib.call('elfi_b200_dist_euclid_thr_f64_host', dev.context(), dev.ptr(S), ld, B, D,
              dev.ptr(obs), dev.ptr(W), K, dev.ptr(thr), dev.ptr(d), dev.ptr(idx),
              ctypes.byref(n) if thr is not None else None)
    if d is not None and K == 1 and (w is None or np.ndim(w) == 1):
        d = d.reshape(B)
    return d, (idx[:n.value] if idx is not None else None)


def _ld(t):
    return t.stride(0) if t.shape[0] > 1 else t.shape[1]


def autocov(x, lags=(1,), out=None):
    x = _matrix(x)
    B, n = x.shape
    lags_arr = np.ascontiguousarray(np.atleast_1d(lags), dtype=np.int32)
    for lag in lags_arr:
        if not 1 <= lag < n:
            raise ValueError('lag {} outside [1, {})'.format(lag, n))
    if out is None:
        out = dev.empty((B, len(lags_arr)))
    _lib.call('elfi_b200_summary_autocov_f64', dev.context(), dev.ptr(x), _ld(x), B, n,
              dev.ptr(lags_arr), len(lags_arr), dev.ptr(out), out.stride(0) if B > 1 else
              out.shape[1], dev.stream_ptr())
    return out


def meanvar(y, out=None):
    y = _matrix(y)
    B, n = y.shape
    if out is None:
        out = dev.empty((B, 2))
    _lib.call('elfi_b200_summary_meanvar_f64', dev.context(), dev.ptr(y), _ld(y), B, n,
              dev.ptr(out), out.stride(0) if B > 1 else out.shape[1], 0, 1, dev.stream_ptr())
    return out


def argsort(keys, return_keys=False):
    keys = dev.to_device(keys).reshape(-1)
    n = keys.numel()
    perm = dev.empty((n,), dtype=torch.int32)
    ks = dev.empty((n,)) if return_keys else None
    _lib.call('elfi_b200_sort_pairs_f64', dev.context(), dev.ptr(keys), n, dev.ptr(ks),
              dev.ptr(perm), dev.stream_ptr())
    return (perm, ks) if return_keys else perm


def _as_2d(t):
    if t.dim() == 2:
        return t
    width = 1
    for extent in t.shape[1:]:
        width *= int(extent)
    return t.reshape(t.shape[0], width)


def take_rows(src, idx):
    src = dev.to_device(src)
    shape = src.shape
    s2 = _as_2d(src)
    if s2.stride(-1) != 1 and s2.shape[1] > 0:
        s2 = s2.contiguous()
    idx = dev.to_device(idx, dtype=torch.int32)
    n = idx.numel()
    width = s2.shape[1]
    dst = dev.empty((n, width))
    if n and width:
        _lib.call('elfi_b200_gather_rows_f64', dev.context(), dev.ptr(s2), _ld(s2), dev.ptr(idx),
                  n, width, dev.ptr(dst), width, dev.stream_ptr())
    return dst.reshape((n,) + tuple(shape[1:]))


def take_rows2(a, b, perm, n_out, map_b=None):
    shape = a.shape if a is not None else b.shape
    a2 = _as_2d(a) if a is not None else None
    b2 = _as_2d(b) if b is not None else None
    width = (a2 if a2 is not None else b2).shape[1]
    n_a = a2.shape[0] if a2 is not None else 0
    dst = dev.empty((n_out, width))
    if n_out and width:
        _lib.call('elfi_b200_gather2_rows_f64', dev.context(), dev.ptr(a2),
                  _ld(a2) if a2 is not None else width, n_a, dev.ptr(b2),
                  _ld(b2) if b2 is not None else width, dev.ptr(map_b), dev.ptr(perm), n_out,
                  width, dev.ptr(dst), width, dev.stream_ptr())
    return dst.reshape((n_out,) + tuple(shape[1:]))


def merge_topn(state, batch, key_state, key_batch, map_b, n_keep):
    if map_b is not None and map_b.dtype != torch.int32:
        raise TypeError('map_b must be an int32 device array of batch row indices')
    n_a = int(key_state.shape[0])
    n_b = int(map_b.numel()) if map_b is not None else int(key_batch.shape[0])
    a2 = [_as_2d(t) for t in state]
    b2 = [_as_2d(dev.to_device(t)) for t in batch]
    widths = [t.shape[1] for t in b2]
    outs = [dev.empty((n_keep, w)) for w in widths]
    n = len(outs)
    if n_keep and n:
        arr_p, arr_i = ctypes.c_void_p * n, ctypes.c_int64 * n
        pa = arr_p(*[t.data_ptr() if n_a else 0 for t in a2])
        la = arr_i(*[_ld(t) if n_a else w for t, w in zip(a2, widths)])
        pb = arr_p(*[t.data_ptr() for t in b2])
        lb = arr_i(*[_ld(t) for t in b2])
        wd = arr_i(*widths)
        pd = arr_p(*[t.data_ptr() for t in outs])
        ld = arr_i(*widths)
        cast = lambda a: ctypes.cast(a, ctypes.c_void_p)
        _lib.call('elfi_b200_topn_merge_f64', dev.context(), dev.ptr(key_state) if n_a else None,
                  key_state.stride(0) if n_a > 1 else 1, n_a, dev.ptr(key_batch),
                  key_batch.stride(0) if key_batch.shape[0] > 1 else 1, dev.ptr(map_b), n_b,
                  n_keep, n, cast(pa), cast(la), cast(pb), cast(lb), cast(wd), cast(pd), cast(ld),
                  dev.stream_ptr())
    return [o.reshape((n_keep,) + tuple(t.shape[1:])) for o, t in zip(outs, batch)]


class CandidateBuffer:

    def __init__(self, capacity, widths):
        self.widths = [int(w) for w in widths]
        self.width = sum(self.widths)
        self.capacity = int(capacity)
        self.rows = dev.empty((self.capacity, self.width))
        self._counters = dev.zeros((2,), dtype=torch.int64)
        self.count = self._counters[0:1]
        self.dropped = self._counters[1:2]

    def reset(self):
        self._counters.zero_()

    def _descriptors(self, sources):
        key = tuple((t.data_ptr(), tuple(t.shape), t.stride(0)) for t in sources)
        cached = getattr(self, '_desc', None)
        if cached is not None and cached[0] == key:
            return cached[1]
        srcs = [_as_2d(t) for t in sources]
        if [t.shape[1] for t in srcs] != self.widths:
            raise ValueError('source widths do not match the buffer layout')
        n = len(srcs)
        ptrs = (ctypes.c_void_p * n)(*[t.data_ptr() for t in srcs])
        lds = (ctypes.c_int64 * n)(*[_ld(t) for t in srcs])
        wid = (ctypes.c_int64 * n)(*self.widths)
        desc = (n, ptrs, lds, wid, ctypes.cast(ptrs, ctypes.c_void_p),
                ctypes.cast(lds, ctypes.c_void_p), ctypes.cast(wid, ctypes.c_void_p),
                dev.ptr(self.rows), dev.ptr(self.count), dev.ptr(self.dropped))
        self._desc = (key, desc)
        return desc

    def append(self, sources, acc_idx, n_acc, max_rows):
        n, _, _, _, pp, pl, pw, prow, pcount, pdrop = self._descriptors(sources)
        _lib.call('elfi_b200_accept_append_f64', dev.context(), dev.ptr(acc_idx), dev.ptr(n_acc),
                  int(max_rows), n, pp, pl, pw, prow, self.width, self.capacity, pcount, pdrop,
                  dev.stream_ptr())

    def bind_batch(self, S, obs, thresholds, d_out, acc_idx, n_acc, extras, w=None):
        S = _matrix(S)
        B, D = S.shape
        W = None if w is None else dev.to_device(w).reshape(-1, D)
        K = 1 if W is None else W.shape[0]
        extras = [_as_2d(t) for t in extras]
        if [K] + [t.shape[1] for t in extras] != self.widths:
            raise ValueError('d / extra widths do not match the buffer layout')
        thr_dev = thresholds if dev.is_device_array(thresholds) else None
        thr_host = None if thr_dev is not None else np.ascontiguousarray(
            np.atleast_1d(thresholds), dtype=np.float64)
        n = len(extras)
        ptrs = (ctypes.c_void_p * max(n, 1))(*[t.data_ptr() for t in extras])
        lds = (ctypes.c_int64 * max(n, 1))(*[_ld(t) for t in extras])
        wid = (ctypes.c_int64 * max(n, 1))(*[t.shape[1] for t in extras])
        keep = (S, obs, W, thr_dev, thr_host, d_out, acc_idx, n_acc, extras, ptrs, lds, wid)
        args = (dev.context(), dev.ptr(S), S.stride(0) if B > 1 else D, B, D, dev.ptr(obs),
                dev.ptr(W), K, dev.ptr(thr_host), dev.ptr(thr_dev), dev.ptr(d_out),
                dev.ptr(acc_idx), dev.ptr(n_acc), n, ctypes.cast(ptrs, ctypes.c_void_p),
                ctypes.cast(lds, ctypes.c_void_p), ctypes.cast(wid, ctypes.c_void_p),
                dev.ptr(self.rows), self.width, self.capacity, dev.ptr(self.count),
                dev.ptr(self.dropped))

        def run(_keep=keep):
            _lib.call('elfi_b200_rejection_batch_f64', *args, dev.stream_ptr())
        return run

    def best(self, n, key_col=0):
        count, dropped = (int(v) for v in self._counters.cpu().tolist())
        keys = self.rows[:count, key_col].contiguous()
        perm = argsort(keys)
        return take_rows(self.rows, perm[:min(n, count)]), count, dropped


def allgather_particles(blocks):
    n = len(blocks)
    blocks = [b.contiguous() for b in blocks]
    rows = blocks[0].shape[0]
    width = int(np.prod(blocks[0].shape[1:])) if blocks[0].dim() > 1 else 1
    if any(tuple(b.shape) != tuple(blocks[0].shape) or b.dtype != torch.float64 for b in blocks):
        raise ValueError('blocks must be fp64 tensors of equal shape')
    outs, streams, ctxs = [], [], []
    for b in blocks:
        with torch.cuda.device(b.device):
            outs.append(torch.empty((n * rows,) + tuple(b.shape[1:]), dtype=torch.float64,
                                    device=b.device))
            streams.append(torch.cuda.current_stream(b.device).cuda_stream)
            ctxs.append(dev.context(b.device).value)
    arr = ctypes.c_void_p * n
    _lib.call('elfi_b200_allgather_particles', ctypes.cast(arr(*ctxs), ctypes.c_void_p), n,
              ctypes.cast(arr(*[b.data_ptr() for b in blocks]), ctypes.c_void_p), rows, width,
              ctypes.cast(arr(*[o.data_ptr() for o in outs]), ctypes.c_void_p),
              ctypes.cast(arr(*streams), ctypes.c_void_p))
    return outs


def weighted_sample_quantile(x, alpha, weights=None):
    x = dev.to_device(x).reshape(-1)
    w = None if weights is None else dev.to_device(weights).reshape(-1)
    if w is not None and w.numel() != x.numel():
        raise ValueError('x and weights must have the same length')
    out = dev.empty((2,))
    _lib.call('elfi_b200_wquantile_f64', dev.context(), dev.ptr(x), dev.ptr(w), x.numel(),
              float(alpha), dev.ptr(out), dev.stream_ptr())
    return float(out[0].item())


def colmoments(S):
    S = _matrix(S)
    B, D = S.shape
    out = dev.empty((2, D))
    _lib.call('elfi_b200_colmoments_f64', dev.context(), dev.ptr(S), _ld(S), B, D, dev.ptr(out),
              dev.stream_ptr())
    out = out.cpu().numpy()
    return out[0], out[1]


def weighted_stats(x, weights=None):
    x = _matrix(x)
    N, p = x.shape
    w = None if weights is None else dev.to_device(weights).reshape(-1)
    stats = dev.empty((2 + 2 * p,))
    _lib.call('elfi_b200_weighted_stats_f64', dev.context(), dev.ptr(x), _ld(x), dev.ptr(w), N, p,
              dev.ptr(stats), dev.stream_ptr())
    s = stats.cpu().numpy()
    return s[0], s[1], s[2:2 + p].copy(), s[2 + p:2 + 2 * p].copy()


def weighted_var(x, weights=None):
    return weighted_stats(x, weights)[3]


def gm_logpdf(x, means, cov=1, weights=None, validate=True, mixed=False):
    means = _matrix(means)
    M, p = means.shape
    x = dev.to_device(x)
    x = x.reshape(-1, p) if x.dim() != 2 else x
    x = _matrix(x)
    N = x.shape[0]
    cov = np.atleast_2d(np.asarray(cov, dtype=np.float64))
    if cov.shape == (1, 1) and p > 1:
        cov = np.eye(p) * cov[0, 0]
    L = np.linalg.cholesky(cov)
    Linv = np.ascontiguousarray(np.linalg.inv(L))
    logdet = 2.0 * float(np.sum(np.log(np.diag(L))))
    w = None if weights is None else dev.to_device(weights).reshape(-1)
    if w is not None and validate:
        if bool((w < 0).any()):
            raise ValueError("Weights must be positive")
        if float(w.sum()) == 0:
            raise ValueError("All weights are zero")
    logq = dev.empty((N,))
    _lib.call('elfi_b200_gm_logpdf_mixed_f64' if mixed else 'elfi_b200_gm_logpdf_f64',
              dev.context(), dev.ptr(x), _ld(x), N, dev.ptr(means),
              _ld(means), dev.ptr(w), M, p, dev.ptr(Linv), logdet, dev.ptr(logq), dev.stream_ptr())
    return logq


def smc_weights(logprior, logq):
    lp = dev.to_device(logprior).reshape(-1)
    lq = dev.to_device(logq).reshape(-1)
    w = dev.empty((lp.numel(),))
    _lib.call('elfi_b200_smc_weights_f64', dev.context(), dev.ptr(lp), dev.ptr(lq), lp.numel(),
              dev.ptr(w), dev.stream_ptr())
    return w


def prior_ma2(batch_size, seed, offset=0, t1=None, which='both'):
    mode = {'both': 0, 't1': 1, 't2': 2}[which]
    if mode == 2:
        t1 = dev.to_device(t1).reshape(-1).contiguous()
        batch_size = t1.numel()
    else:
        t1 = dev.empty((batch_size,))
    t2 = dev.empty((batch_size,)) if mode != 1 else None
    _lib.call('elfi_b200_prior_ma2_f64', dev.context(), batch_size, int(seed), int(offset), mode,
              dev.ptr(t1), dev.ptr(t2), dev.stream_ptr())
    return (t1, t2) if mode == 0 else (t1 if mode == 1 else t2)


def logprior_ma2(params):
    x = _matrix(params)
    out = dev.empty((x.shape[0],))
    _lib.call('elfi_b200_logprior_ma2_f64', dev.context(), dev.ptr(x), _ld(x), x.shape[0],
              dev.ptr(out), dev.stream_ptr())
    return out


def sim_ma2(t1, t2, n_obs=100, seed=0, offset=0, want_data=False, want_summaries=True):
    t1 = dev.to_device(t1).reshape(-1)
    t2 = dev.to_device(t2).reshape(-1)
    B = t1.numel()
    X = dev.empty((B, n_obs)) if want_data else None
    S = dev.empty((B, 2)) if want_summaries else None
    _lib.call('elfi_b200_sim_ma2_f64', dev.context(), dev.ptr(t1), dev.ptr(t2), B, n_obs,
              int(seed), int(offset), dev.ptr(X), n_obs, dev.ptr(S), 2, dev.stream_ptr())
    return X, S


def gm_cdf(weights, n=None):
    w = None if weights is None else dev.to_device(weights).reshape(-1)
    n = int(w.numel()) if w is not None else int(n)
    cumw = dev.empty((n,))
    _lib.call('elfi_b200_gm_cdf_f64', dev.context(), dev.ptr(w), n, dev.ptr(cumw), dev.stream_ptr())
    return cumw


def gm_rvs(means, cov, weights, size, seed, offset=0, support=0, box=None, cdf=None):
    means = _matrix(means)
    N, p = means.shape
    cov = np.atleast_2d(np.asarray(cov, dtype=np.float64))
    if cov.shape == (1, 1) and p > 1:
        cov = np.eye(p) * cov[0, 0]
    L = np.ascontiguousarray(np.linalg.cholesky(cov))
    boxarr = None
    if support == 2:
        boxarr = np.ascontiguousarray(np.concatenate([np.asarray(box[0], dtype=np.float64),
                                                      np.asarray(box[1], dtype=np.float64)]))
    out = dev.empty((size, p))
    if cdf is None:
        cdf = gm_cdf(weights, N)
    elif cdf.numel() != N:
        raise ValueError('cdf must have one entry per mixture component')
    _lib.call('elfi_b200_gm_rvs_cdf_f64', dev.context(), dev.ptr(means), _ld(means), dev.ptr(cdf), N,
              p, dev.ptr(L), size, int(seed), int(offset), int(support), dev.ptr(boxarr),
              dev.ptr(out), p, dev.stream_ptr())
    return out


def _gauss_prm(prm):
    return np.ascontiguousarray(prm, dtype=np.float64)


def prior_gauss(batch_size, seed, prm, offset=0):
    mu, sigma = dev.empty((batch_size,)), dev.empty((batch_size,))
    _lib.call('elfi_b200_prior_gauss_f64', dev.context(), batch_size, int(seed), int(offset),
              dev.ptr(_gauss_prm(prm)), dev.ptr(mu), dev.ptr(sigma), dev.stream_ptr())
    return mu, sigma


def logprior_gauss(params, prm):
    x = _matrix(params)
    out = dev.empty((x.shape[0],))
    _lib.call('elfi_b200_logprior_gauss_f64', dev.context(), dev.ptr(x), _ld(x), x.shape[0],
              dev.ptr(_gauss_prm(prm)), dev.ptr(out), dev.stream_ptr())
    return out


def sim_gauss(mu, sigma, n_obs=50, seed=0, offset=0, want_data=False, want_summaries=True):
    mu = dev.to_device(mu).reshape(-1).contiguous()
    sigma = dev.to_device(sigma).reshape(-1).contiguous()
    B = mu.numel()
    Y = dev.empty((B, n_obs)) if want_data else None
    S = dev.empty((B, 2)) if want_summaries else None
    _lib.call('elfi_b200_sim_gauss_f64', dev.context(), dev.ptr(mu), dev.ptr(sigma), B, n_obs,
              int(seed), int(offset), dev.ptr(Y), n_obs, dev.ptr(S), 2, dev.stream_ptr())
    return Y, S


def sim_gnk(A, B, g, k, n_obs=50, seed=0, offset=0, c=0.8):
    cols = [dev.to_device(v).reshape(-1).contiguous() for v in (A, B, g, k)]
    n = cols[0].numel()
    if any(col.numel() != n for col in cols):
        raise ValueError('A, B, g and k must have the same number of elements')
    Y = dev.empty((n, n_obs))
    _lib.call('elfi_b200_sim_gnk_f64', dev.context(), dev.ptr(cols[0]), dev.ptr(cols[1]),
              dev.ptr(cols[2]), dev.ptr(cols[3]), float(c), n, n_obs, int(seed), int(offset),
              dev.ptr(Y), n_obs, dev.stream_ptr())
    return Y


def logprior_box(params, lo, width):
    x = _matrix(params)
    p = x.shape[1]
    box = np.ascontiguousarray(np.concatenate([np.broadcast_to(np.asarray(lo, dtype=np.float64), (p,)),
                                               np.broadcast_to(np.asarray(width, dtype=np.float64), (p,))]))
    out = dev.empty((x.shape[0],))
    _lib.call('elfi_b200_logprior_box_f64', dev.context(), dev.ptr(x), _ld(x), x.shape[0], p,
              dev.ptr(box), dev.ptr(out), dev.stream_ptr())
    return out


def kliep_fit(x, y, weights_x=None, weights_y=None, sigma=1.0, n_basis=100, epsilon=0.001,
              max_iter=200, abs_tol=0.01, conv_check_interval=20):
    x = _matrix(x)
    y = _matrix(y)
    if x.shape[0] < n_basis:
        raise ValueError("Number of RBFs ({}) can't be larger than number of samples ({}).".format(
            n_basis, x.shape[0]))
    wx = None if weights_x is None else dev.to_device(weights_x).reshape(-1)
    wy = None if weights_y is None else dev.to_device(weights_y).reshape(-1)
    alpha = dev.empty((n_basis,))
    res = (ctypes.c_double * 2)()
    dev.synchronize()
    _lib.call('elfi_b200_kliep_fit_f64', dev.context(), dev.ptr(x), _ld(x), x.shape[0], dev.ptr(y),
              _ld(y), y.shape[0], x.shape[1], dev.ptr(wx), dev.ptr(wy), float(sigma), int(n_basis),
              float(epsilon), int(max_iter), float(abs_tol), int(conv_check_interval),
              dev.ptr(alpha), res)
    return alpha, float(res[0]), int(res[1])


def rowsort(x):
    x = _matrix(x)
    B, n = x.shape
    out = dev.empty((B, n))
    _lib.call('elfi_b200_rowsort_f64', dev.context(), dev.ptr(x), _ld(x), B, n, dev.ptr(out), n,
              dev.stream_ptr())
    return out
```

Baseline: 26.58 million.

## Fuse mask compaction and accepted-row append into the distance launch path

Measured after the change: 27.70 million, median of 6. 4.2% higher.

```diff
diff --git a/elfi_b200/csrc/accept.cuh b/elfi_b200/csrc/accept.cuh
--- /dev/null
+++ b/elfi_b200/csrc/accept.cuh
@@ -0,0 +1,179 @@
+#pragma once
+
+#include <cooperative_groups.h>
+
+#include "common.cuh"
+
+namespace elfi {
+
+constexpr int APPEND_MAX_SRC = 8;
+struct AppendSources {
+    const double* ptr[APPEND_MAX_SRC];
+    int64_t ld[APPEND_MAX_SRC];
+    int32_t width[APPEND_MAX_SRC];
+    int32_t col0[APPEND_MAX_SRC];
+    int32_t n_src, total_width;
+};
+
+struct AcceptTail {
+    int32_t* idx;
+    int64_t* n_out;
+    AppendSources src;
+    double* dst;
+    int64_t ld_dst;
+    int64_t capacity;
+    int64_t* count;
+    int64_t* dropped;
+    int64_t* cta_counts;
+    __host__ __device__ bool active() const { return idx != nullptr || n_out != nullptr; }
+};
+
+__device__ __forceinline__ int64_t block_sum_i64(int64_t v, int64_t* ws) {
+    const int lane = threadIdx.x & 31, wid = threadIdx.x >> 5;
+    for (int o = 16; o > 0; o >>= 1) v += __shfl_xor_sync(0xffffffffu, v, o);
+    if (lane == 0) ws[wid] = v;
+    __syncthreads();
+    if (threadIdx.x == 0) {
+        int64_t t = 0;
+        for (int i = 0; i < int(blockDim.x >> 5); ++i) t += ws[i];
+        ws[32] = t;
+    }
+    __syncthreads();
+    const int64_t t = ws[32];
+    __syncthreads();
+    return t;
+}
+
+__device__ __forceinline__ int64_t block_excl_scan(int v, int64_t* ws, int64_t* total) {
+    const int lane = threadIdx.x & 31, wid = threadIdx.x >> 5;
+    int incl = v;
+    for (int o = 1; o < 32; o <<= 1) {
+        const int t = __shfl_up_sync(0xffffffffu, incl, o);
+        if (lane >= o) incl += t;
+    }
+    if (lane == 31) ws[wid] = incl;
+    __syncthreads();
+    if (wid == 0) {
+        const int64_t w = lane < int(blockDim.x >> 5) ? ws[lane] : 0;
+        int64_t inc2 = w;
+        for (int o = 1; o < 32; o <<= 1) {
+            const int64_t t = __shfl_up_sync(0xffffffffu, inc2, o);
+            if (lane >= o) inc2 += t;
+        }
+        ws[lane] = inc2 - w;
+        if (lane == 31) ws[32] = inc2;
+    }
+    __syncthreads();
+    const int64_t r = ws[wid] + (incl - v);
+    *total = ws[32];
+    __syncthreads();
+    return r;
+}
+
+__device__ __forceinline__ int64_t mask_prefix_bits(const uint32_t* mask, int64_t lo) {
+    constexpr int U = 8;
+    int64_t before = 0;
+    const int64_t nv = (reinterpret_cast<uintptr_t>(mask) & 15) == 0 ? (lo >> 2) : 0;
+    const uint4* m4 = reinterpret_cast<const uint4*>(mask);
+    for (int64_t v0 = threadIdx.x; v0 < nv; v0 += U * int64_t(blockDim.x)) {
+        uint4 q[U];
+#pragma unroll
+        for (int u = 0; u < U; ++u) {
+            const int64_t v = v0 + int64_t(u) * blockDim.x;
+            q[u] = v < nv ? __ldcg(m4 + v) : make_uint4(0u, 0u, 0u, 0u);
+        }
+#pragma unroll
+        for (int u = 0; u < U; ++u)
+            before += __popc(q[u].x) + __popc(q[u].y) + __popc(q[u].z) + __popc(q[u].w);
+    }
+    for (int64_t w = (nv << 2) + threadIdx.x; w < lo; w += blockDim.x) before += __popc(__ldcg(mask + w));
+    return before;
+}
+
+__device__ __forceinline__ int64_t compact_words(const uint32_t* mask, int64_t lo, int64_t hi,
+                                                 int64_t base, int32_t* idx, int64_t* ws) {
+    for (int64_t w0 = lo; w0 < hi; w0 += blockDim.x) {
+        const int64_t w = w0 + threadIdx.x;
+        uint32_t bits = w < hi ? __ldcg(mask + w) : 0u;
+        int64_t total;
+        int64_t pos = base + block_excl_scan(__popc(bits), ws, &total);
+        if (idx != nullptr) {
+            while (bits) {
+                const int bit = __ffs(bits) - 1;
+                bits &= bits - 1;
+                idx[pos++] = int32_t(w * 32 + bit);
+            }
+        }
+        base += total;
+    }
+    return base;
+}
+
+__device__ __forceinline__ void append_rows(const int32_t* acc_idx, int64_t j0, int64_t j1,
+                                            const AppendSources& src, double* dst, int64_t ld_dst,
+                                            int64_t base, int64_t t0, int64_t stride) {
+    const int64_t total = (j1 - j0) * src.total_width;
+    for (int64_t t = t0; t < total; t += stride) {
+        const int64_t jj = t / src.total_width;
+        const int c = int(t - jj * src.total_width);
+        const int64_t j = j0 + jj;
+        const int64_t row = acc_idx ? int64_t(acc_idx[j]) : j;
+        int k = 0;
+#pragma unroll
+        for (int q = 1; q < APPEND_MAX_SRC; ++q)
+            if (q < src.n_src && c >= src.col0[q]) k = q;
+        dst[(base + j) * ld_dst + c] = __ldcg(src.ptr[k] + row * src.ld[k] + (c - src.col0[k]));
+    }
+}
+
+__device__ __forceinline__ void accept_count(int64_t n_acc, int64_t capacity, int64_t* count,
+                                             int64_t* dropped) {
+    int64_t room = capacity - *count;
+    if (room < 0) room = 0;
+    const int64_t rows = n_acc < room ? n_acc : room;
+    if (dropped) *dropped += n_acc - rows;
+    *count += rows;
+}
+
+__device__ __forceinline__ void accept_tail(const AcceptTail& t, const uint32_t* mask, int64_t B,
+                                            int64_t* ws) {
+    cooperative_groups::grid_group grid = cooperative_groups::this_grid();
+    int64_t fill = 0;
+    if (t.dst != nullptr) fill = *t.count;
+    grid.sync();
+    const int64_t nwords = (B + 31) / 32;
+    const int64_t per = (nwords + gridDim.x - 1) / gridDim.x;
+    int64_t lo = int64_t(blockIdx.x) * per;
+    if (lo > nwords) lo = nwords;
+    const int64_t hi = lo + per < nwords ? lo + per : nwords;
+    int64_t mine = 0;
+    for (int64_t w = lo + threadIdx.x; w < hi; w += blockDim.x) mine += __popc(__ldcg(mask + w));
+    mine = block_sum_i64(mine, ws);
+    if (threadIdx.x == 0) t.cta_counts[blockIdx.x] = mine;
+    grid.sync();
+    int64_t before = 0;
+    for (int64_t c = threadIdx.x; c < blockIdx.x; c += blockDim.x) before += __ldcg(t.cta_counts + c);
+    const int64_t j0 = block_sum_i64(before, ws);
+    const int64_t j1 = compact_words(mask, lo, hi, j0, t.idx, ws);
+    if (t.dst != nullptr) {
+        int64_t room = t.capacity - fill;
+        if (room < 0) room = 0;
+        __syncthreads();
+        append_rows(t.idx, j0, j1 < room ? j1 : room, t.src, t.dst, t.ld_dst, fill, threadIdx.x,
+                    blockDim.x);
+    }
+    if (blockIdx.x == gridDim.x - 1 && threadIdx.x == 0) {
+        if (t.n_out != nullptr) *t.n_out = j1;
+        if (t.dst != nullptr) accept_count(j1, t.capacity, t.count, t.dropped);
+    }
+}
+
+int launch_accept_append(elfi_b200_ctx* ctx, const int32_t* acc_idx, const int64_t* n_acc,
+                         int64_t max_rows, const AppendSources& src, double* dst, int64_t ld_dst,
+                         int64_t capacity, int64_t* count, int64_t* dropped, cudaStream_t stream);
+int dist_thr_accept(elfi_b200_ctx* ctx, const double* S, int64_t ldS, int64_t B, int64_t D,
+                    const double* obs, const double* W, int64_t K, const double* thr_host,
+                    const double* thr_dev, double* d_out, AcceptTail tail,
+                    cudaStream_t stream);
+
+}
diff --git a/elfi_b200/csrc/distance.cu b/elfi_b200/csrc/distance.cu
--- a/elfi_b200/csrc/distance.cu
+++ b/elfi_b200/csrc/distance.cu
@@ -18,6 +18,7 @@
     double* mom_partial;
     const double* thr_dev;
     double thr[ELFI_B200_MAX_NESTED];
+    AcceptTail accept;
     __device__ __forceinline__ double threshold(int k) const {
         return thr_dev ? __ldg(thr_dev + k) : thr[k];
     }
@@ -339,62 +340,16 @@
 }
 
 __global__ void __launch_bounds__(1024)
-compact_mask_kernel(const uint32_t* __restrict__ mask, int64_t nwords, int64_t B,
-                    int32_t* __restrict__ idx, int64_t* __restrict__ n_out) {
-    __shared__ int64_t warp_sums[32];
-    __shared__ int64_t base_s;
-    const int tid = threadIdx.x;
-    const int lane = tid & 31;
-    const int wid = tid >> 5;
-    const int64_t first = int64_t(blockIdx.x) * 1024;
-
-    int64_t before = 0;
-    for (int64_t w = tid; w < first; w += 1024) before += __popc(mask[w]);
-    for (int o = 16; o > 0; o >>= 1) before += __shfl_xor_sync(0xffffffffu, before, o);
-    if (lane == 0) warp_sums[wid] = before;
-    __syncthreads();
-    if (tid == 0) {
-        int64_t t = 0;
-        for (int i = 0; i < 32; ++i) t += warp_sums[i];
-        base_s = t;
-    }
-    __syncthreads();
-    const int64_t base = base_s;
-    __syncthreads();
-
-    const int64_t w = first + tid;
-    const uint32_t bits = w < nwords ? mask[w] : 0u;
-    const int cnt = __popc(bits);
-    int incl = cnt;
-    for (int o = 1; o < 32; o <<= 1) {
-        const int t = __shfl_up_sync(0xffffffffu, incl, o);
-        if (lane >= o) incl += t;
-    }
-    if (lane == 31) warp_sums[wid] = incl;
-    __syncthreads();
-    if (wid == 0) {
-        int64_t v = warp_sums[lane];
-        int64_t inc2 = v;
-        for (int o = 1; o < 32; o <<= 1) {
-            const int64_t t = __shfl_up_sync(0xffffffffu, inc2, o);
-            if (lane >= o) inc2 += t;
-        }
-        warp_sums[lane] = inc2 - v;
-        if (lane == 31 && blockIdx.x == gridDim.x - 1 && n_out != nullptr) *n_out = base + inc2;
-    }
-    __syncthreads();
-    int64_t pos = base + warp_sums[wid] + (incl - cnt);
-    if (idx != nullptr) {
-        uint32_t b = bits;
-        while (b) {
-            const int bit = __ffs(b) - 1;
-            b &= b - 1;
-            idx[pos++] = int32_t(w * 32 + bit);
-        }
-    }
-}
-
-int launch_compact_mask(const uint32_t* mask, int64_t B, int32_t* idx, int64_t* n_out,
+compact_mask_kernel(const uint32_t* mask, int64_t nwords, int32_t* idx, int64_t* n_out) {
+    __shared__ int64_t ws[33];
+    const int64_t lo = int64_t(blockIdx.x) * 1024;
+    const int64_t hi = lo + 1024 < nwords ? lo + 1024 : nwords;
+    const int64_t base = block_sum_i64(mask_prefix_bits(mask, lo), ws);
+    const int64_t end = compact_words(mask, lo, hi, base, idx, ws);
+    if (threadIdx.x == 0 && blockIdx.x == gridDim.x - 1 && n_out != nullptr) *n_out = end;
+}
+
+static int launch_compact_mask(const uint32_t* mask, int64_t B, int32_t* idx, int64_t* n_out,
                         cudaStream_t stream) {
     const int64_t nwords = (B + 31) / 32;
     if (nwords == 0) {
@@ -402,15 +357,23 @@
         return ELFI_B200_OK;
     }
     const unsigned blocks = unsigned((nwords + 1023) / 1024);
-    compact_mask_kernel<<<blocks, 1024, 0, stream>>>(mask, nwords, B, idx, n_out);
+    compact_mask_kernel<<<blocks, 1024, 0, stream>>>(mask, nwords, idx, n_out);
     ELFI_CUDA_OK(cudaGetLastError());
     return ELFI_B200_OK;
+}
+
+static int launch_accept_standalone(elfi_b200_ctx* ctx, const uint32_t* mask, int64_t B,
+                                    const AcceptTail& t, cudaStream_t stream) {
+    int rc = launch_compact_mask(mask, B, t.idx, t.n_out, stream);
+    if (rc || t.dst == nullptr) return rc;
+    return launch_accept_append(ctx, t.idx, t.n_out, B, t.src, t.dst, t.ld_dst, t.capacity, t.count,
+                                t.dropped, stream);
 }
 
 int launch_dist(elfi_b200_ctx* ctx, const double* S, int64_t ldS, int64_t B, int64_t D,
                 const double* obs, const double* W, int64_t K, const double* thr_host,
                 double* d_out, uint32_t* mask, cudaStream_t stream,
-                const double* thr_dev = nullptr) {
+                const double* thr_dev = nullptr, const AcceptTail* tail = nullptr) {
     DistParams p;
     memset(&p, 0, sizeof(p));
     p.obs = obs;
@@ -422,7 +385,9 @@
     p.thr_dev = thr_dev;
     if (thr_host)
         for (int k = 0; k < K; ++k) p.thr[k] = thr_host[k];
-    if (B == 0) return ELFI_B200_OK;
+    if (tail) p.accept = *tail;
+    if (B == 0) return p.accept.active() ? launch_accept_standalone(ctx, mask, B, p.accept, stream)
+                                         : ELFI_B200_OK;
 
     const int64_t Dp = ((D + RS_BOX_COLS - 1) / RS_BOX_COLS) * RS_BOX_COLS;
     const bool use_tma = D >= RS_BOX_COLS && tma_compatible(S, ldS);
@@ -444,7 +409,7 @@
     const unsigned blocks = unsigned((B + 255) / 256);
     dist_direct_kernel<<<blocks, 256, 0, stream>>>(S, ldS, B, int(D), p);
     ELFI_CUDA_OK(cudaGetLastError());
-    return ELFI_B200_OK;
+    return p.accept.active() ? launch_accept_standalone(ctx, mask, B, p.accept, stream) : ELFI_B200_OK;
 }
 
 struct MetricParams : DistParams {
@@ -531,12 +496,14 @@
         return rowstream_launch<MetricConsumer<METRIC>>(ctx, S, ldS, B, D, aux, p, stream);
     metric_direct_kernel<METRIC><<<unsigned((B + 255) / 256), 256, 0, stream>>>(S, ldS, B, int(D), p);
     ELFI_CUDA_OK(cudaGetLastError());
-    return ELFI_B200_OK;
+    return p.accept.active() ? launch_accept_standalone(ctx, p.mask, B, p.accept, stream)
+                             : ELFI_B200_OK;
 }
 
 static int launch_metric(elfi_b200_ctx* ctx, int metric, double pexp, const double* S, int64_t ldS,
                          int64_t B, int64_t D, const double* obs, const double* thr_host,
-                         double* d_out, uint32_t* mask, cudaStream_t stream) {
+                         double* d_out, uint32_t* mask, const AcceptTail& tail,
+                         cudaStream_t stream) {
     MetricParams p;
     memset(&p, 0, sizeof(p));
     p.obs = obs;
@@ -546,7 +513,8 @@
     p.has_thr = thr_host != nullptr;
     if (thr_host) p.thr[0] = thr_host[0];
     p.pexp = pexp;
-    if (B == 0) return ELFI_B200_OK;
+    p.accept = tail;
+    if (B == 0) return tail.active() ? launch_accept_standalone(ctx, mask, B, tail, stream) : ELFI_B200_OK;
     switch (metric) {
         case ELFI_B200_METRIC_SQEUCLIDEAN:
             return launch_metric_t<ELFI_B200_METRIC_SQEUCLIDEAN>(ctx, S, ldS, B, D, p, stream);
@@ -659,7 +627,8 @@
 
 static int launch_seuclid(elfi_b200_ctx* ctx, const double* S, int64_t ldS, int64_t B, int64_t D,
                           const double* obs, const double* V, const double* thr_host,
-                          double* d_out, uint32_t* mask, cudaStream_t stream) {
+                          double* d_out, uint32_t* mask, const AcceptTail& tail,
+                          cudaStream_t stream) {
     MetricParams p;
     memset(&p, 0, sizeof(p));
     p.obs = obs;
@@ -669,14 +638,15 @@
     p.K = 1;
     p.has_thr = thr_host != nullptr;
     if (thr_host) p.thr[0] = thr_host[0];
-    if (B == 0) return ELFI_B200_OK;
+    p.accept = tail;
+    if (B == 0) return tail.active() ? launch_accept_standalone(ctx, mask, B, tail, stream) : ELFI_B200_OK;
     const int64_t Dp = ((D + RS_BOX_COLS - 1) / RS_BOX_COLS) * RS_BOX_COLS;
     const size_t aux = size_t(Dp) * 8 * 2;
     if (D >= RS_BOX_COLS && tma_compatible(S, ldS) && rs_pick_stages(ctx->smem_optin, aux) >= 2)
         return rowstream_launch<SeuclidConsumer>(ctx, S, ldS, B, D, aux, p, stream);
     seuclid_direct_kernel<<<unsigned((B + 255) / 256), 256, 0, stream>>>(S, ldS, B, int(D), p);
     ELFI_CUDA_OK(cudaGetLastError());
-    return ELFI_B200_OK;
+    return tail.active() ? launch_accept_standalone(ctx, mask, B, tail, stream) : ELFI_B200_OK;
 }
 
 static int check_dist_args(const void* S, int64_t ldS, int64_t B, int64_t D, const void* obs,
@@ -693,6 +663,40 @@
     return ELFI_B200_OK;
 }
 
+static uint8_t* accept_scratch(elfi_b200_ctx* ctx, int64_t B, size_t extra, AcceptTail* tail) {
+    const size_t mask_bytes = (size_t((B + 31) / 32) * 4 + 255) & ~size_t(255);
+    uint8_t* base = static_cast<uint8_t*>(
+        ctx_scratch(ctx, mask_bytes + extra + size_t(ctx->sm_count) * 8 + 256));
+    if (base) tail->cta_counts = reinterpret_cast<int64_t*>(base + mask_bytes + extra);
+    return base;
+}
+
+int dist_thr_accept(elfi_b200_ctx* ctx, const double* S, int64_t ldS, int64_t B, int64_t D,
+                    const double* obs, const double* W, int64_t K, const double* thr_host,
+                    const double* thr_dev, double* d_out, AcceptTail tail,
+                    cudaStream_t stream) {
+    const void* thr = thr_host ? static_cast<const void*>(thr_host) : thr_dev;
+    int rc = check_dist_args(S, ldS, B, D, obs, W, K, thr, tail.idx);
+    if (rc) return rc;
+    ELFI_REQUIRE(B == 0 || d_out != nullptr, "dist: d_out is NULL");
+    ELFI_CUDA_OK(cudaSetDevice(ctx->device));
+    uint32_t* mask = nullptr;
+    if (thr != nullptr) {
+        mask = reinterpret_cast<uint32_t*>(accept_scratch(ctx, B, 0, &tail));
+        if (!mask) return ELFI_B200_ERR_NOMEM;
+    }
+    return launch_dist(ctx, S, ldS, B, D, obs, W, K, thr_host, d_out, mask, stream, thr_dev,
+                       thr != nullptr ? &tail : nullptr);
+}
+
+static AcceptTail indices_tail(int32_t* acc_idx, int64_t* n_acc) {
+    AcceptTail t;
+    memset(&t, 0, sizeof(t));
+    t.idx = acc_idx;
+    t.n_out = n_acc;
+    return t;
+}
+
 }
 
 extern "C" {
@@ -703,22 +707,8 @@
                                   int64_t* n_acc, void* stream_) {
     using namespace elfi;
     ELFI_REQUIRE(ctx != nullptr, "dist: ctx is NULL");
-    int rc = check_dist_args(S, ldS, B, D, obs, W, K, thr_host, acc_idx);
-    if (rc) return rc;
-    ELFI_REQUIRE(B == 0 || d_out != nullptr, "dist: d_out is NULL");
-    cudaStream_t stream = static_cast<cudaStream_t>(stream_);
-    ELFI_CUDA_OK(cudaSetDevice(ctx->device));
-    uint32_t* mask = nullptr;
-    if (thr_host != nullptr) {
-        const size_t nwords = size_t((B + 31) / 32);
-        mask = static_cast<uint32_t*>(ctx_scratch(ctx, nwords * 4 + 256));
-        if (!mask) return ELFI_B200_ERR_NOMEM;
-    }
-    rc = launch_dist(ctx, S, ldS, B, D, obs, W, K, thr_host, d_out, mask, stream);
-    if (rc) return rc;
-    if (thr_host != nullptr && (acc_idx != nullptr || n_acc != nullptr))
-        return launch_compact_mask(mask, B, acc_idx, n_acc, stream);
-    return ELFI_B200_OK;
+    return dist_thr_accept(ctx, S, ldS, B, D, obs, W, K, thr_host, nullptr, d_out,
+                           indices_tail(acc_idx, n_acc), static_cast<cudaStream_t>(stream_));
 }
 
 int elfi_b200_dist_euclid_thr_dev_f64(elfi_b200_ctx* ctx, const double* S, int64_t ldS, int64_t B,
@@ -727,19 +717,8 @@
                                       int64_t* n_acc, void* stream_) {
     using namespace elfi;
     ELFI_REQUIRE(ctx != nullptr && thr_dev != nullptr, "dist: ctx or thr_dev is NULL");
-    int rc = check_dist_args(S, ldS, B, D, obs, W, K, thr_dev, acc_idx);
-    if (rc) return rc;
-    ELFI_REQUIRE(B == 0 || d_out != nullptr, "dist: d_out is NULL");
-    cudaStream_t stream = static_cast<cudaStream_t>(stream_);
-    ELFI_CUDA_OK(cudaSetDevice(ctx->device));
-    const size_t nwords = size_t((B + 31) / 32);
-    uint32_t* mask = static_cast<uint32_t*>(ctx_scratch(ctx, nwords * 4 + 256));
-    if (!mask) return ELFI_B200_ERR_NOMEM;
-    rc = launch_dist(ctx, S, ldS, B, D, obs, W, K, nullptr, d_out, mask, stream, thr_dev);
-    if (rc) return rc;
-    if (acc_idx != nullptr || n_acc != nullptr)
-        return launch_compact_mask(mask, B, acc_idx, n_acc, stream);
-    return ELFI_B200_OK;
+    return dist_thr_accept(ctx, S, ldS, B, D, obs, W, K, nullptr, thr_dev, d_out,
+                           indices_tail(acc_idx, n_acc), static_cast<cudaStream_t>(stream_));
 }
 
 int elfi_b200_dist_euclid_mom_f64(elfi_b200_ctx* ctx, const double* S, int64_t ldS, int64_t B,
@@ -762,16 +741,13 @@
                        rs_pick_stages(ctx->smem_optin, aux) >= 2;
     const size_t mask_bytes = (size_t((B + 31) / 32) * 4 + 255) & ~size_t(255);
     const size_t part_bytes = fused ? size_t(ctx->sm_count) * 16 * 2 * D * 8 : 0;
-    uint8_t* base = static_cast<uint8_t*>(ctx_scratch(ctx, mask_bytes + part_bytes + 256));
+    AcceptTail tail = thr ? indices_tail(acc_idx, n_acc) : indices_tail(nullptr, nullptr);
+    uint8_t* base = accept_scratch(ctx, B, part_bytes, &tail);
     if (!base) return ELFI_B200_ERR_NOMEM;
     uint32_t* mask = thr ? reinterpret_cast<uint32_t*>(base) : nullptr;
     if (!fused) {
-        rc = launch_dist(ctx, S, ldS, B, D, obs, W, K, thr_host, d_out, mask, stream, thr_dev);
+        rc = launch_dist(ctx, S, ldS, B, D, obs, W, K, thr_host, d_out, mask, stream, thr_dev, &tail);
         if (rc) return rc;
-        if (thr && (acc_idx != nullptr || n_acc != nullptr)) {
-            rc = launch_compact_mask(mask, B, acc_idx, n_acc, stream);
-            if (rc) return rc;
-        }
         return elfi_b200_colmoments_f64(ctx, S, ldS, B, D, moments, stream_);
     }
     DistParams p;
@@ -787,16 +763,13 @@
         for (int k = 0; k < K; ++k) p.thr[k] = thr_host[k];
     p.shift_src = S;
     p.mom_partial = reinterpret_cast<double*>(base + mask_bytes);
-    if (K <= 2) rc = launch_nested_moments<2>(ctx, S, ldS, B, D, p, moments, stream);
-    else if (K <= 4) rc = launch_nested_moments<4>(ctx, S, ldS, B, D, p, moments, stream);
-    else if (K <= 6) rc = launch_nested_moments<6>(ctx, S, ldS, B, D, p, moments, stream);
-    else if (K <= 8) rc = launch_nested_moments<8>(ctx, S, ldS, B, D, p, moments, stream);
-    else if (K <= 16) rc = launch_nested_moments<16>(ctx, S, ldS, B, D, p, moments, stream);
-    else rc = launch_nested_moments<32>(ctx, S, ldS, B, D, p, moments, stream);
-    if (rc) return rc;
-    if (thr && (acc_idx != nullptr || n_acc != nullptr))
-        return launch_compact_mask(mask, B, acc_idx, n_acc, stream);
-    return ELFI_B200_OK;
+    p.accept = tail;
+    if (K <= 2) return launch_nested_moments<2>(ctx, S, ldS, B, D, p, moments, stream);
+    if (K <= 4) return launch_nested_moments<4>(ctx, S, ldS, B, D, p, moments, stream);
+    if (K <= 6) return launch_nested_moments<6>(ctx, S, ldS, B, D, p, moments, stream);
+    if (K <= 8) return launch_nested_moments<8>(ctx, S, ldS, B, D, p, moments, stream);
+    if (K <= 16) return launch_nested_moments<16>(ctx, S, ldS, B, D, p, moments, stream);
+    return launch_nested_moments<32>(ctx, S, ldS, B, D, p, moments, stream);
 }
 
 int elfi_b200_dist_euclid_thr_f64_host(elfi_b200_ctx* ctx, const double* S_host, int64_t ldS,
@@ -903,16 +876,14 @@
     ELFI_REQUIRE(B == 0 || d_out != nullptr, "dist_metric: d_out is NULL");
     cudaStream_t stream = static_cast<cudaStream_t>(stream_);
     ELFI_CUDA_OK(cudaSetDevice(ctx->device));
+    AcceptTail tail = thr_host ? indices_tail(acc_idx, n_acc) : indices_tail(nullptr, nullptr);
     uint32_t* mask = nullptr;
     if (thr_host != nullptr) {
-        mask = static_cast<uint32_t*>(ctx_scratch(ctx, size_t((B + 31) / 32) * 4 + 256));
+        mask = reinterpret_cast<uint32_t*>(accept_scratch(ctx, B, 0, &tail));
         if (!mask) return ELFI_B200_ERR_NOMEM;
     }
-    rc = launch_metric(ctx, int(metric), pexp, S, ldS, B, D, obs, thr_host, d_out, mask, stream);
-    if (rc) return rc;
-    if (thr_host != nullptr && (acc_idx != nullptr || n_acc != nullptr))
-        return launch_compact_mask(mask, B, acc_idx, n_acc, stream);
-    return ELFI_B200_OK;
+    return launch_metric(ctx, int(metric), pexp, S, ldS, B, D, obs, thr_host, d_out, mask, tail,
+                         stream);
 }
 
 int elfi_b200_dist_seuclidean_thr_f64(elfi_b200_ctx* ctx, const double* S, int64_t ldS, int64_t B,
@@ -927,16 +898,13 @@
     ELFI_REQUIRE(B == 0 || d_out != nullptr, "dist_seuclidean: d_out is NULL");
     cudaStream_t stream = static_cast<cudaStream_t>(stream_);
     ELFI_CUDA_OK(cudaSetDevice(ctx->device));
+    AcceptTail tail = thr_host ? indices_tail(acc_idx, n_acc) : indices_tail(nullptr, nullptr);
     uint32_t* mask = nullptr;
     if (thr_host != nullptr) {
-        mask = static_cast<uint32_t*>(ctx_scratch(ctx, size_t((B + 31) / 32) * 4 + 256));
+        mask = reinterpret_cast<uint32_t*>(accept_scratch(ctx, B, 0, &tail));
         if (!mask) return ELFI_B200_ERR_NOMEM;
     }
-    rc = launch_seuclid(ctx, S, ldS, B, D, obs, V, thr_host, d_out, mask, stream);
-    if (rc) return rc;
-    if (thr_host != nullptr && (acc_idx != nullptr || n_acc != nullptr))
-        return launch_compact_mask(mask, B, acc_idx, n_acc, stream);
-    return ELFI_B200_OK;
-}
-
-}
+    return launch_seuclid(ctx, S, ldS, B, D, obs, V, thr_host, d_out, mask, tail, stream);
+}
+
+}
diff --git a/elfi_b200/csrc/rowstream.cuh b/elfi_b200/csrc/rowstream.cuh
--- a/elfi_b200/csrc/rowstream.cuh
+++ b/elfi_b200/csrc/rowstream.cuh
@@ -1,7 +1,9 @@
 #pragma once
 
 #include <type_traits>
+#include <utility>
 
+#include "accept.cuh"
 #include "common.cuh"
 
 namespace elfi {
@@ -10,6 +12,9 @@
 template <class C> struct rs_has_tile_info<C, std::void_t<decltype(C::RS_TILE_INFO)>> : std::true_type {};
 template <class C, class = void> struct rs_has_finish : std::false_type {};
 template <class C> struct rs_has_finish<C, std::void_t<decltype(C::RS_FINISH)>> : std::true_type {};
+template <class P, class = void> struct rs_has_accept : std::false_type {};
+template <class P> struct rs_has_accept<P, std::void_t<decltype(std::declval<P>().accept)>>
+    : std::true_type {};
 
 constexpr int RS_WARPS = 8;
 constexpr int RS_BOX_ROWS = 32;
@@ -110,6 +115,10 @@
         __syncwarp();
         c.finish(gw, lane);
     }
+    if constexpr (rs_has_accept<typename Consumer::Params>::value) {
+        if (params.accept.active())
+            accept_tail(params.accept, params.mask, B, reinterpret_cast<int64_t*>(smem));
+    }
 }
 
 template <class Consumer, int WARPS = RS_WARPS>
@@ -132,6 +141,27 @@
     const int64_t ntiles = (B + RS_BOX_ROWS - 1) / RS_BOX_ROWS;
     int64_t ctas = (ntiles + WARPS - 1) / WARPS;
     if (ctas > ctx->sm_count) ctas = ctx->sm_count;
+    if constexpr (rs_has_accept<typename Consumer::Params>::value) {
+        if (params.accept.active()) {
+            int per_sm = 0;
+            ELFI_CUDA_OK(cudaOccupancyMaxActiveBlocksPerMultiprocessor(&per_sm, kern, WARPS * 32,
+                                                                       smem_bytes));
+            ELFI_REQUIRE(per_sm >= 1, "row stream: no CTA fits on an SM (smem %zu bytes)", smem_bytes);
+            if (ctas > int64_t(per_sm) * ctx->sm_count) ctas = int64_t(per_sm) * ctx->sm_count;
+            cudaLaunchConfig_t cfg = {};
+            cudaLaunchAttribute attr[1];
+            attr[0].id = cudaLaunchAttributeCooperative;
+            attr[0].val.cooperative = 1;
+            cfg.gridDim = dim3(unsigned(ctas));
+            cfg.blockDim = dim3(WARPS * 32);
+            cfg.dynamicSmemBytes = smem_bytes;
+            cfg.stream = stream;
+            cfg.attrs = attr;
+            cfg.numAttrs = 1;
+            ELFI_CUDA_OK(cudaLaunchKernelEx(&cfg, kern, map, B, int(D), ns, params));
+            return ELFI_B200_OK;
+        }
+    }
     kern<<<dim3(unsigned(ctas)), dim3(WARPS * 32), smem_bytes, stream>>>(map, B, int(D), ns, params);
     ELFI_CUDA_OK(cudaGetLastError());
     return ELFI_B200_OK;
diff --git a/elfi_b200/csrc/select.cu b/elfi_b200/csrc/select.cu
--- a/elfi_b200/csrc/select.cu
+++ b/elfi_b200/csrc/select.cu
@@ -1,11 +1,14 @@
 #include <cstdlib>
 
+#include "accept.cuh"
 #include "eqweight.h"
 #include "pairwise.cuh"
 
 namespace elfi {
 
-constexpr int SORT_CHUNK = 1024;
+static int sort_chunk(int64_t n) {
+    return n <= (int64_t(1) << 18) ? 256 : n <= (int64_t(1) << 19) ? 512 : 1024;
+}
 constexpr int SORT_WARPS = 8;
 
 __device__ __forceinline__ uint64_t key_to_u64(double d) {
@@ -44,7 +47,7 @@
 }
 
 __global__ void __launch_bounds__(SORT_WARPS * 32)
-sort_upsweep_kernel(const uint64_t* __restrict__ ukeys, int64_t n, int pass, int64_t nw,
+sort_upsweep_kernel(const uint64_t* __restrict__ ukeys, int64_t n, int pass, int64_t nw, int chunk,
                     const uint32_t* __restrict__ ghist, uint32_t* __restrict__ whist) {
     if (pass_trivial(ghist, pass, n, ukeys[0])) return;
     __shared__ uint32_t h[SORT_WARPS][256];
@@ -53,8 +56,8 @@
     for (int i = lane; i < 256; i += 32) h[warp][i] = 0;
     __syncwarp();
     if (gw < nw) {
-        const int64_t lo = gw * SORT_CHUNK;
-        const int64_t hi = (lo + SORT_CHUNK < n) ? lo + SORT_CHUNK : n;
+        const int64_t lo = gw * chunk;
+        const int64_t hi = (lo + chunk < n) ? lo + chunk : n;
         for (int64_t i = lo + lane; i < hi; i += 32)
             atomicAdd(&h[warp][(ukeys[i] >> (8 * pass)) & 255], 1u);
         __syncwarp();
@@ -104,14 +107,14 @@
 
 __global__ void __launch_bounds__(SORT_WARPS * 32)
 sort_scatter_kernel(const uint64_t* __restrict__ kin, const int32_t* __restrict__ vin, int64_t n,
-                    int pass, int64_t nw, const uint32_t* __restrict__ ghist,
+                    int pass, int64_t nw, int chunk, const uint32_t* __restrict__ ghist,
                     const uint32_t* __restrict__ whist, uint64_t* __restrict__ kout,
                     int32_t* __restrict__ vout) {
     const int warp = threadIdx.x >> 5, lane = threadIdx.x & 31;
     const int64_t gw = int64_t(blockIdx.x) * SORT_WARPS + warp;
     if (gw >= nw) return;
-    const int64_t lo = gw * SORT_CHUNK;
-    const int64_t hi = (lo + SORT_CHUNK < n) ? lo + SORT_CHUNK : n;
+    const int64_t lo = gw * chunk;
+    const int64_t hi = (lo + chunk < n) ? lo + chunk : n;
     if (pass_trivial(ghist, pass, n, kin[0])) {
         for (int64_t i = lo + lane; i < hi; i += 32) {
             kout[i] = kin[i];
@@ -158,19 +161,21 @@
     uint32_t* ghist;
     uint32_t* whist;
     int64_t nw;
+    int chunk;
 };
 
 static size_t align256(size_t v) { return (v + 255) & ~size_t(255); }
 
 static size_t sort_scratch_bytes(int64_t n) {
-    const int64_t nw = (n + SORT_CHUNK - 1) / SORT_CHUNK;
+    const int64_t nw = (n + sort_chunk(n) - 1) / sort_chunk(n);
     return 2 * align256(size_t(n) * 8) + 2 * align256(size_t(n) * 4) + align256(8 * 256 * 4) +
            align256(size_t(256) * nw * 4);
 }
 
 static SortScratch carve_sort(uint8_t* base, int64_t n) {
     SortScratch s;
-    s.nw = (n + SORT_CHUNK - 1) / SORT_CHUNK;
+    s.chunk = sort_chunk(n);
+    s.nw = (n + s.chunk - 1) / s.chunk;
     size_t o = 0;
     for (int i = 0; i < 2; ++i) { s.k[i] = reinterpret_cast<uint64_t*>(base + o); o += align256(size_t(n) * 8); }
     for (int i = 0; i < 2; ++i) { s.v[i] = reinterpret_cast<int32_t*>(base + o); o += align256(size_t(n) * 4); }
@@ -189,10 +194,11 @@
     const unsigned wblocks = unsigned((s.nw + SORT_WARPS - 1) / SORT_WARPS);
     int cur = 0;
     for (int pass = 0; pass < 8; ++pass) {
-        sort_upsweep_kernel<<<wblocks, SORT_WARPS * 32, 0, stream>>>(s.k[cur], n, pass, s.nw, s.ghist, s.whist);
+        sort_upsweep_kernel<<<wblocks, SORT_WARPS * 32, 0, stream>>>(s.k[cur], n, pass, s.nw,
+                                                                     s.chunk, s.ghist, s.whist);
         sort_scan_kernel<<<256, 1024, 0, stream>>>(s.k[cur], n, pass, s.nw, s.ghist, s.whist);
         sort_scatter_kernel<<<wblocks, SORT_WARPS * 32, 0, stream>>>(
-            s.k[cur], s.v[cur], n, pass, s.nw, s.ghist, s.whist, s.k[cur ^ 1], s.v[cur ^ 1]);
+            s.k[cur], s.v[cur], n, pass, s.nw, s.chunk, s.ghist, s.whist, s.k[cur ^ 1], s.v[cur ^ 1]);
         cur ^= 1;
     }
     ELFI_CUDA_OK(cudaGetLastError());
@@ -210,44 +216,52 @@
     }
 }
 
-constexpr int APPEND_MAX_SRC = 8;
-struct AppendSources {
-    const double* ptr[APPEND_MAX_SRC];
-    int64_t ld[APPEND_MAX_SRC];
-    int32_t width[APPEND_MAX_SRC];
-    int32_t col0[APPEND_MAX_SRC];
-    int32_t n_src, total_width;
-};
-
 __global__ void __launch_bounds__(256)
-accept_append_kernel(const int32_t* __restrict__ acc_idx, const int64_t* __restrict__ n_acc,
-                     AppendSources src, double* __restrict__ dst, int64_t ld_dst, int64_t capacity,
-                     const int64_t* __restrict__ count) {
+accept_append_kernel(const int32_t* acc_idx, const int64_t* n_acc, AppendSources src, double* dst,
+                     int64_t ld_dst, int64_t capacity, const int64_t* count) {
     const int64_t base = *count;
     int64_t room = capacity - base;
     if (room < 0) room = 0;
     const int64_t rows = *n_acc < room ? *n_acc : room;
-    const int64_t total = rows * src.total_width;
-    const int64_t stride = int64_t(gridDim.x) * blockDim.x;
-    for (int64_t t = int64_t(blockIdx.x) * blockDim.x + threadIdx.x; t < total; t += stride) {
-        const int64_t j = t / src.total_width;
-        const int c = int(t - j * src.total_width);
-        const int64_t row = acc_idx ? int64_t(acc_idx[j]) : j;
-        int k = 0;
-#pragma unroll
-        for (int q = 1; q < APPEND_MAX_SRC; ++q)
-            if (q < src.n_src && c >= src.col0[q]) k = q;
-        dst[(base + j) * ld_dst + c] = src.ptr[k][row * src.ld[k] + (c - src.col0[k])];
-    }
-}
-
-__global__ void accept_count_kernel(const int64_t* __restrict__ n_acc, int64_t capacity,
-                                    int64_t* __restrict__ count, int64_t* __restrict__ dropped) {
-    int64_t room = capacity - *count;
-    if (room < 0) room = 0;
-    const int64_t rows = *n_acc < room ? *n_acc : room;
-    if (dropped) *dropped += *n_acc - rows;
-    *count += rows;
+    append_rows(acc_idx, 0, rows, src, dst, ld_dst, base,
+                int64_t(blockIdx.x) * blockDim.x + threadIdx.x, int64_t(gridDim.x) * blockDim.x);
+}
+
+__global__ void accept_count_kernel(const int64_t* n_acc, int64_t capacity, int64_t* count,
+                                    int64_t* dropped) {
+    accept_count(*n_acc, capacity, count, dropped);
+}
+
+int launch_accept_append(elfi_b200_ctx* ctx, const int32_t* acc_idx, const int64_t* n_acc,
+                         int64_t max_rows, const AppendSources& src, double* dst, int64_t ld_dst,
+                         int64_t capacity, int64_t* count, int64_t* dropped, cudaStream_t stream) {
+    if (max_rows == 0) return ELFI_B200_OK;
+    int64_t blocks = (max_rows * src.total_width + 255) / 256;
+    if (blocks > int64_t(ctx->sm_count) * 8) blocks = int64_t(ctx->sm_count) * 8;
+    accept_append_kernel<<<unsigned(blocks), 256, 0, stream>>>(acc_idx, n_acc, src, dst, ld_dst,
+                                                              capacity, count);
+    accept_count_kernel<<<1, 1, 0, stream>>>(n_acc, capacity, count, dropped);
+    ELFI_CUDA_OK(cudaGetLastError());
+    return ELFI_B200_OK;
+}
+
+static int pack_sources(int64_t n_src, const double* const* src_host, const int64_t* ld_src_host,
+                        const int64_t* width_host, int64_t ld_dst, AppendSources* src) {
+    memset(src, 0, sizeof(*src));
+    src->n_src = int32_t(n_src);
+    int64_t col = 0;
+    for (int k = 0; k < n_src; ++k) {
+        ELFI_REQUIRE(src_host[k] && width_host[k] >= 1 && ld_src_host[k] >= width_host[k],
+                     "accept_append: bad source %d", k);
+        src->ptr[k] = src_host[k];
+        src->ld[k] = ld_src_host[k];
+        src->width[k] = int32_t(width_host[k]);
+        src->col0[k] = int32_t(col);
+        col += width_host[k];
+    }
+    ELFI_REQUIRE(col <= ld_dst && col < (int64_t(1) << 30), "accept_append: ld_dst < total width");
+    src->total_width = int32_t(col);
+    return ELFI_B200_OK;
 }
 
 __global__ void __launch_bounds__(256)
@@ -779,38 +793,13 @@
     ELFI_REQUIRE(n_src >= 1 && n_src <= APPEND_MAX_SRC, "accept_append: 1..%d sources", APPEND_MAX_SRC);
     ELFI_REQUIRE(max_rows >= 0 && capacity >= 0, "accept_append: bad shape");
     AppendSources src;
-    memset(&src, 0, sizeof(src));
-    src.n_src = int32_t(n_src);
-    int64_t col = 0;
-    for (int k = 0; k < n_src; ++k) {
-        ELFI_REQUIRE(src_host[k] && width_host[k] >= 1 && ld_src_host[k] >= width_host[k],
-                     "accept_append: bad source %d", k);
-        src.ptr[k] = src_host[k];
-        src.ld[k] = ld_src_host[k];
-        src.width[k] = int32_t(width_host[k]);
-        src.col0[k] = int32_t(col);
-        col += width_host[k];
-    }
-    ELFI_REQUIRE(col <= ld_dst && col < (int64_t(1) << 30), "accept_append: ld_dst < total width");
-    src.total_width = int32_t(col);
+    int rc = pack_sources(n_src, src_host, ld_src_host, width_host, ld_dst, &src);
+    if (rc) return rc;
     if (max_rows == 0) return ELFI_B200_OK;
-    cudaStream_t stream = static_cast<cudaStream_t>(stream_);
     ELFI_CUDA_OK(cudaSetDevice(ctx->device));
-    int64_t blocks = (max_rows * col + 255) / 256;
-    if (blocks > int64_t(ctx->sm_count) * 8) blocks = int64_t(ctx->sm_count) * 8;
-    accept_append_kernel<<<unsigned(blocks), 256, 0, stream>>>(acc_idx, n_acc, src, dst, ld_dst,
-                                                              capacity, count);
-    accept_count_kernel<<<1, 1, 0, stream>>>(n_acc, capacity, count, dropped);
-    ELFI_CUDA_OK(cudaGetLastError());
-    return ELFI_B200_OK;
-}
-
-extern "C" int elfi_b200_dist_euclid_thr_f64(elfi_b200_ctx*, const double*, int64_t, int64_t, int64_t,
-                                             const double*, const double*, int64_t, const double*,
-                                             double*, int32_t*, int64_t*, void*);
-extern "C" int elfi_b200_dist_euclid_thr_dev_f64(elfi_b200_ctx*, const double*, int64_t, int64_t,
-                                                 int64_t, const double*, const double*, int64_t,
-                                                 const double*, double*, int32_t*, int64_t*, void*);
+    return launch_accept_append(ctx, acc_idx, n_acc, max_rows, src, dst, ld_dst, capacity, count,
+                                dropped, static_cast<cudaStream_t>(stream_));
+}
 
 int elfi_b200_rejection_batch_f64(elfi_b200_ctx* ctx, const double* S, int64_t ldS, int64_t B,
                                   int64_t D, const double* obs, const double* W, int64_t K,
@@ -826,12 +815,7 @@
                  "rejection_batch: thresholds on the host OR on the device");
     ELFI_REQUIRE(n_extra >= 0 && n_extra < APPEND_MAX_SRC, "rejection_batch: 0..%d extra sources",
                  APPEND_MAX_SRC - 1);
-    int rc = thr_host
-        ? elfi_b200_dist_euclid_thr_f64(ctx, S, ldS, B, D, obs, W, K, thr_host, d_out, acc_idx, n_acc,
-                                        stream_)
-        : elfi_b200_dist_euclid_thr_dev_f64(ctx, S, ldS, B, D, obs, W, K, thr_dev, d_out, acc_idx,
-                                            n_acc, stream_);
-    if (rc) return rc;
+    ELFI_REQUIRE(dst && count && capacity >= 0, "accept_append: NULL argument or bad shape");
     const double* src[APPEND_MAX_SRC];
     int64_t ld[APPEND_MAX_SRC], width[APPEND_MAX_SRC];
     src[0] = d_out; ld[0] = K; width[0] = K;
@@ -840,8 +824,19 @@
         ld[k + 1] = ld_extra_host[k];
         width[k + 1] = width_extra_host[k];
     }
-    return elfi_b200_accept_append_f64(ctx, acc_idx, n_acc, B, n_extra + 1, src, ld, width, dst,
-                                       ld_dst, capacity, count, dropped, stream_);
+    AcceptTail tail;
+    memset(&tail, 0, sizeof(tail));
+    int rc = pack_sources(n_extra + 1, src, ld, width, ld_dst, &tail.src);
+    if (rc) return rc;
+    tail.idx = acc_idx;
+    tail.n_out = n_acc;
+    tail.dst = dst;
+    tail.ld_dst = ld_dst;
+    tail.capacity = capacity;
+    tail.count = count;
+    tail.dropped = dropped;
+    return dist_thr_accept(ctx, S, ldS, B, D, obs, W, K, thr_host, thr_dev, d_out, tail,
+                           static_cast<cudaStream_t>(stream_));
 }
 
 int elfi_b200_wquantile_f64(elfi_b200_ctx* ctx, const double* x, const double* w, int64_t n,
diff --git a/elfi_b200/ops.py b/elfi_b200/ops.py
--- a/elfi_b200/ops.py
+++ b/elfi_b200/ops.py
@@ -356,10 +356,21 @@
         return run
 
     def best(self, n, key_col=0):
+        if not 0 <= key_col < self.width:
+            raise IndexError('key column {} outside the {} columns'.format(key_col, self.width))
+        n = max(0, min(int(n), self.capacity))
+        out = dev.empty((n, self.width))
+        w = self.width
+        arr_p, arr_i = ctypes.c_void_p * 1, ctypes.c_int64 * 1
+        arrays = (arr_p(self.rows.data_ptr()), arr_i(w), arr_p(0), arr_i(w), arr_i(w),
+                  arr_p(out.data_ptr()), arr_i(w))
+        head = (dev.context(), ctypes.c_void_p(self.rows.data_ptr() + 8 * key_col), w)
+        tail = [ctypes.cast(a, ctypes.c_void_p) for a in arrays] + [dev.stream_ptr()]
         count, dropped = (int(v) for v in self._counters.cpu().tolist())
-        keys = self.rows[:count, key_col].contiguous()
-        perm = argsort(keys)
-        return take_rows(self.rows, perm[:min(n, count)]), count, dropped
+        n_keep = min(n, count)
+        if n_keep:
+            _lib.call('elfi_b200_topn_merge_f64', *head, count, None, 1, None, 0, n_keep, 1, *tail)
+        return out[:n_keep], count, dropped
 
 
 def allgather_particles(blocks):
```
